# carlos-gg/dl4ds

Measured on AMD Instinct MI355X. Metric: HR samples/s (train step) at 4x 128->512 residual SR, higher is better.
Workload: dtype f32; 1 GPU; configs[1]: net_postupsampling(resnet, spc, scale=4, lr 128x128 -> hr 512x512, 204405 params), MAE, Adam; per_gpu_batch=64, global_batch=64, parallelism=dp1

## Files before the change

dl4ds_amd/csrc/capi.cpp:

```cpp
#include "../../include/dl4ds_hip.h"
#include "graph.h"
#include "runtime.h"
#include "dist.h"
#include "prof.h"
#include <algorithm>
#include <cmath>
#include <cstring>
#include <cstdlib>
#include <mutex>
#include <vector>

Trainer* trainer_create(Graph* g, int loss_kind, const AdamCfg& cfg);
void graph_load_inputs(Graph& g, const float* const* inputs, int n_inputs, int B, bool is_host);
void trainer_evaluate(Trainer& t, const float* const* inputs, int n_inputs, const float* y_true, int B, bool is_host);
void trainer_loss_and_grads(Trainer& t, const float* const* inputs, int n_inputs, const float* y_true, int B, bool is_host,
                            bool reduce_across_ranks);
void trainer_step(Trainer& t, const float* const* inputs, int n_inputs, const float* y_true, int B, bool is_host, float* loss_host);
struct CganTrainer;
CganTrainer* cgan_create(Graph* gen, Graph* disc, int px_loss_kind, float lr, float beta1, float lam);
void cgan_destroy(CganTrainer* t);
void cgan_step(CganTrainer& t, const float* const* gen_inputs, int n_gen_inputs, const float* hr, int B, bool is_host,
               const float* dropout_keep_host, bool apply_update, float* losses_host);
Trainer* cgan_disc_trainer(CganTrainer* t);
Trainer* cgan_gen_trainer(CganTrainer* t);
// ... 169 lines not shown
    API_END
}
int dl4ds_memcpy_d2d(void* dst, const void* src, size_t bytes) {
    API_BEGIN
    HIP_CHECK(hipMemcpyAsync(dst, src, bytes, hipMemcpyDeviceToDevice, S()));
    API_END
}
int dl4ds_memset(void* p, int value, size_t bytes) {
    API_BEGIN
    HIP_CHECK(hipMemsetAsync(p, value, bytes, S()));
    API_END
}
int dl4ds_sync(void) {
    API_BEGIN
    dist_stream_sync(S(), "dl4ds_sync");
    API_END
}
namespace {
__global__ void raise_device_error_kernel(unsigned* word, unsigned code) {
    __hip_atomic_fetch_or(word, code, __ATOMIC_RELAXED, __HIP_MEMORY_SCOPE_SYSTEM);
}
}
int dl4ds_debug_raise_device_error(int code) {
    API_BEGIN
    hipLaunchKernelGGL(raise_device_error_kernel, dim3(1), dim3(1), 0, S(), device_error_word(), (unsigned)code);
    HIP_CHECK(hipGetLastError());
    API_END
}
int dl4ds_event_timer_start(void) {
    API_BEGIN
    HIP_CHECK(hipEventRecord(rt().ev0, S()));
    API_END
}
int dl4ds_event_timer_stop(float* ms) {
    API_BEGIN
    HIP_CHECK(hipEventRecord(rt().ev1, S()));
    HIP_CHECK(hipEventSynchronize(rt().ev1));
    HIP_CHECK(hipEventElapsedTime(ms, rt().ev0, rt().ev1));
    API_END
}

int dl4ds_profile_enable(int on) {
    API_BEGIN
    HIP_CHECK(hipStreamSynchronize(S()));
    prof().reset();
    prof().on = (on != 0);
    API_END
}
int dl4ds_profile_filter(const char* tag_prefix) {
    API_BEGIN
    prof().filter = tag_prefix ? tag_prefix : "";
    API_END
}
int dl4ds_profile_report(char* buf, size_t buflen) {
    API_BEGIN
    const std::string r = prof().report_json(S());
    DL4DS_REQUIRE(r.size() + 1 <= buflen, "profile report buffer too small");
    std::memcpy(buf, r.c_str(), r.size() + 1);
    API_END
}

int dl4ds_op_conv2d_fwd(const float* x, const float* w, const float* b, const float* add, float* y, int N, int H, int W,
                        int Cin, int Cout, int KS, int relu, int d2s_r) {
    API_BEGIN
    TView in = make_view(nc(x), N, H, W, Cin);
    TView out = (d2s_r > 1) ? make_view_d2s(y, N, H, W, Cout, d2s_r) : make_view(y, N, H, W, Cout);
    ConvEpilogue ep;
    ep.bias = b;
    if (add) ep.add = make_view(nc(add), N, H, W, Cout);
    ep.relu = relu;
    conv2d_forward(S(), in, w, KS, out, ep);
    API_END
}
int dl4ds_op_conv2d_epilogue(const float* x, const float* w, const float* b, const float* add, const float* mask, float* y, int N,
                             int H, int W, int Cin, int Cout, int KS, int relu, int accumulate) {
    API_BEGIN
    ConvEpilogue ep;
    ep.bias = b;
    if (add) ep.add = make_view(nc(add), N, H, W, Cout);
    if (mask) ep.mask = make_view(nc(mask), N, H, W, Cout);
    ep.relu = relu;
    ep.accumulate = accumulate;
    conv2d_forward(S(), make_view(nc(x), N, H, W, Cin), w, KS, make_view(y, N, H, W, Cout), ep);
    API_END
}
int dl4ds_op_conv2d_dgrad(const float* dz, const float* w, float* dx, int N, int H, int W, int Cin, int Cout, int KS,
                          int d2s_r, int accumulate) {
    API_BEGIN
    const size_t nw = (size_t)KS * KS * Cin * Cout;
    float* wt = scratch(nw * sizeof(float));
    conv2d_dgrad_weights(S(), w, wt, KS, Cin, Cout);
    TView dzv = (d2s_r > 1) ? make_view_d2s(nc(dz), N, H, W, Cout, d2s_r) : make_view(nc(dz), N, H, W, Cout);
    ConvEpilogue ep;
    ep.accumulate = accumulate;
    conv2d_forward(S(), dzv, wt, KS, make_view(dx, N, H, W, Cin), ep);
    API_END
}
int dl4ds_op_conv2d_wgrad(const float* x, const float* dz, float* dw, int N, int H, int W, int Cin, int Cout, int KS,
                          int d2s_r, int accumulate) {
    API_BEGIN
    TView xv = make_view(nc(x), N, H, W, Cin);
    TView dzv = (d2s_r > 1) ? make_view_d2s(nc(dz), N, H, W, Cout, d2s_r) : make_view(nc(dz), N, H, W, Cout);
    const size_t ws = conv2d_wgrad_workspace_bytes(xv, dzv, KS);
    conv2d_wgrad(S(), xv, dzv, KS, dw, accumulate, nullptr, 0, scratch(ws), ws);
    API_END
}
int dl4ds_op_bias_act_bwd(float* dy, const float* y, float* db, int N, int H, int W, int C) {
    API_BEGIN
    TView dyv = make_view(dy, N, H, W, C);
    TView none{nullptr, 0, 0, 0, 0, 0, 0, 0};
    const size_t ws = bias_grad_workspace_bytes(dyv);
    bias_act_backward(S(), dyv, y ? make_view(nc(y), N, H, W, C) : none, y ? dyv : none, db, 0, scratch(ws), ws);
    API_END
}
int dl4ds_op_conv2d_transpose_fwd(const float* x, const float* w, float* y, int N, int H, int W, int Cin, int Cout,
                                  int KS, int stride, int relu) {
    API_BEGIN
    TView in = make_view(nc(x), N, H, W, Cin);
    TView out = make_view(y, N, H * stride, W * stride, Cout);
    const size_t ws = conv2d_transpose_workspace_bytes(in, out, KS, stride);
    conv2d_transpose_forward(S(), in, w, KS, stride, out, relu, scratch(ws), ws);
    API_END
}
int dl4ds_op_conv2d_transpose_dgrad(const float* dz, const float* w, float* dx, int N, int H, int W, int Cin, int Cout,
                                    int KS, int stride, int accumulate) {
    API_BEGIN
    TView dxv = make_view(dx, N, H, W, Cin);
    TView dzv = make_view(nc(dz), N, H * stride, W * stride, Cout);
    const size_t ws = conv2d_transpose_workspace_bytes(dxv, dzv, KS, stride);
    conv2d_transpose_dgrad(S(), dzv, w, KS, stride, dxv, accumulate, scratch(ws), ws);
    API_END
}
int dl4ds_op_conv2d_transpose_wgrad(const float* x, const float* dz, float* dw, int N, int H, int W, int Cin, int Cout,
                                    int KS, int stride, int accumulate) {
    API_BEGIN
    TView xv = make_view(nc(x), N, H, W, Cin);
    TView dzv = make_view(nc(dz), N, H * stride, W * stride, Cout);
    const size_t ws = conv2d_transpose_workspace_bytes(xv, dzv, KS, stride);
    conv2d_transpose_wgrad(S(), xv, dzv, KS, stride, dw, accumulate, scratch(ws), ws);
    API_END
}
int dl4ds_batch_prepare(const float* hr, const float* pred, const float* stat, const int* idx_host, const int* cy_host,
                        const int* cx_host, float* out_lr, float* out_hr, float* out_stat, int H, int W, int C, int P, int S_,
                        int T, int B, int scale, int psy, int psx, int pin, int static_in_lr) {
    API_BEGIN
    DL4DS_REQUIRE(B > 0 && idx_host && cy_host && cx_host, "batch_prepare: index lists missing");
    const int* d_idx = upload_index_lists(idx_host, cy_host, cx_host, B);
    batch_prepare(S(), hr, pred, stat, d_idx, d_idx + B, d_idx + 2 * B, out_lr, out_hr, out_stat, H, W, C, P, S_, T, B, scale,
                  psy, psx, pin, static_in_lr);
    API_END
}
int dl4ds_batch_prepare_taps(const float* hr, const float* pred, const float* stat, const int* idx_host, const int* cy_host,
                             const int* cx_host, float* out_lr, float* out_hr, float* out_stat, float* scratch_dev, int H, int W,
                             int C, int P, int S_, int T, int B, int scale, int psy, int psx, int pin, int static_in_lr,
                             const dl4ds_tap_axis* dn_patch, const dl4ds_tap_axis* dn_field, const dl4ds_tap_axis* up_field) {
    API_BEGIN
    DL4DS_REQUIRE(B > 0 && idx_host && cy_host && cx_host, "batch_prepare_taps: index lists missing");
    const int* d_idx = upload_index_lists(idx_host, cy_host, cx_host, B);
    auto axes = [](const dl4ds_tap_axis* t, TapAxis* o) -> const TapAxis* {
        if (!t) return nullptr;
        for (int i = 0; i < 2; ++i) { o[i].idx = t[i].idx; o[i].wt = t[i].wt; o[i].k = t[i].k; }
        return o;
    };
    TapAxis a0[2], a1[2], a2[2];
    batch_prepare_taps(S(), hr, pred, stat, d_idx, d_idx + B, d_idx + 2 * B, out_lr, out_hr, out_stat, scratch_dev, H, W, C, P,
                       S_, T, B, scale, psy, psx, pin, static_in_lr, axes(dn_patch, a0), axes(dn_field, a1), axes(up_field, a2));
// ... 803 lines not shown
```

dl4ds_amd/csrc/conv.hip:

```cpp
#include "ops.h"
#include "prof.h"
#include "conv_kernels.h"
#include "conv_cache.h"
#include <algorithm>
#include <mutex>
#include <vector>
#include <cstdlib>

namespace {

constexpr int kLdsBudget = 80 * 1024;

template <int KS, int MT, int NT, int WM, int WN, int KSP = 1>
__global__ void __launch_bounds__(64 * WM * WN * KSP, KSP > 2 ? 1 : 2) conv_igemm_kernel(const ConvParams a) {
    constexpr int TW = 16;
    constexpr int NTHR = 64 * WM * WN * KSP;
    constexpr int BM = WM * MT * 16;
    constexpr int TH = BM / TW;
    constexpr int BN = WN * NT * 16;
    constexpr int BN4 = BN / 4;
    constexpr int PAD = KS / 2;
    constexpr int TWH = TW + KS - 1;
    constexpr int THH = TH + KS - 1;
    constexpr int HPIX = TWH * THH;
// ... 1296 lines not shown
    constexpr bool PF = (CIT == 1 && WCO == 1 && KS <= 3);
    constexpr int TWH = 16 + KS - 1, THH = 8 + KS - 1, HPIX = TWH * THH;
    constexpr int CIB = 16 * CIT, COB = 16 * COT * WCO;
    constexpr int PX = (CIB % 32 == 16) ? CIB : CIB + 16;
    constexpr int PZ = (COB % 32 == 16) ? COB : COB + 16;
    constexpr int WK = 4 / WCO;
    constexpr size_t red_bytes = (size_t)(WK / 2) * WCO * (KS * KS * CIT * COT * 4 + COT) * 64 * sizeof(float);
    static const bool no_rows = exp_env("DL4DS_NO_WGRAD_ROWS") != nullptr;
    constexpr bool ROWS_OK = (KS == 3 || KS == 1 || (KS == 5 && CIT == 1)) && COT == 1;
    const bool rows = ROWS_OK && !no_rows && ((KS == 3 && !PF) || pl.ws);
    const bool ws = rows && pl.ws;
    const size_t lds = rows ? std::max((size_t)(ws ? 2 : 1) * (HPIX * (CIB + 4) + 128 * (COB + 4)) * sizeof(float), red_bytes)
                            : std::max((size_t)(PF ? 2 : 1) * (HPIX * PX + 128 * PZ) * sizeof(float), red_bytes);
    void (*kern)(const WgradParams) = conv_wgrad_kernel<KS, CIT, COT, WCO, PF>;
    static const bool no_pack = exp_env("DL4DS_NO_WGRAD_PACK") != nullptr;
    constexpr bool PACK_OK = ROWS_OK && CIT == 1 && (KS == 3 || KS == 5);
    const bool pack = PACK_OK && ws && p.Cin <= 8 && !no_pack;
    if constexpr (ROWS_OK) {
        if constexpr (KS == 3) {
            if constexpr (PF) { if (rows) kern = conv_wgrad_rows_ws_kernel<CIT, WCO, 3>; }
            else if (rows) kern = ws ? conv_wgrad_rows_ws_kernel<CIT, WCO, 3> : conv_wgrad_rows_kernel<CIT, WCO>;
        } else {
            if (rows) kern = conv_wgrad_rows_ws_kernel<CIT, WCO, KS>;
        }
    }
    if constexpr (PACK_OK) {
        if (pack) kern = conv_wgrad_rows_ws_kernel<1, WCO, KS, true>;
    }
    static std::once_flag once;
    std::call_once(once, [&]() {
        HIP_CHECK(hipFuncSetAttribute(reinterpret_cast<const void*>(conv_wgrad_kernel<KS, CIT, COT, WCO, PF>),
                                      hipFuncAttributeMaxDynamicSharedMemorySize, KS >= 7 ? kLdsMax : kLdsBudget));
        if constexpr (PACK_OK)
            HIP_CHECK(hipFuncSetAttribute(reinterpret_cast<const void*>(conv_wgrad_rows_ws_kernel<1, WCO, KS, true>),
                                          hipFuncAttributeMaxDynamicSharedMemorySize, kLdsMax));
        if constexpr (ROWS_OK) {
            HIP_CHECK(hipFuncSetAttribute(reinterpret_cast<const void*>(conv_wgrad_rows_ws_kernel<CIT, WCO, KS>),
                                          hipFuncAttributeMaxDynamicSharedMemorySize, kLdsMax));
            if constexpr (KS == 3 && !PF)
                HIP_CHECK(hipFuncSetAttribute(reinterpret_cast<const void*>(conv_wgrad_rows_kernel<CIT, WCO>),
                                              hipFuncAttributeMaxDynamicSharedMemorySize, kLdsBudget));
        }
    });
    DL4DS_REQUIRE(lds <= (size_t)((ws || KS >= 7) ? kLdsMax : kLdsBudget), "wgrad tile does not fit in LDS");
    dim3 grid((unsigned)pl.S, (unsigned)cdiv(p.Cout, COB), (unsigned)cdiv(p.Cin, CIB));
    const double px = (double)p.x.N * p.H * p.W;
    ProfScope ps(s, std::string(rows ? "conv_wgrad_rows<" : "conv_wgrad<") + std::to_string(KS) + "," + std::to_string(CIT) +
                        "," + std::to_string(COT) + "," + std::to_string(WCO) + ">",
                 2.0 * px * KS * KS * p.Cin * p.Cout, 4.0 * (px * (p.Cin + p.Cout) + (double)KS * KS * p.Cin * p.Cout));
    DL4DS_LAUNCH(kern, grid, dim3(ws ? 512 : 256), lds, s, p);
    HIP_CHECK(hipGetLastError());
}

template <int KS, int CIT>
void dispatch_wgrad_wco(hipStream_t s, WgradParams& p, const WgradPlan& pl) {
    switch (pl.WCO) {
        case 1: launch_wgrad<KS, CIT, 1, 1>(s, p, pl); break;
        case 2: launch_wgrad<KS, CIT, 1, 2>(s, p, pl); break;
        default: launch_wgrad<KS, CIT, 1, 4>(s, p, pl); break;
    }
}

template <int KS>
void dispatch_wgrad(hipStream_t s, WgradParams& p, const WgradPlan& pl) {
    switch (pl.CIT) {
        case 3: dispatch_wgrad_wco<KS, 3>(s, p, pl); break;
        case 2: dispatch_wgrad_wco<KS, 2>(s, p, pl); break;
        default: dispatch_wgrad_wco<KS, 1>(s, p, pl); break;
    }
}

}

float* conv_splitk_scratch(hipStream_t s, size_t floats) { return splitk_scratch(s, floats); }
void conv_splitk_combine(hipStream_t s, const float* slabs, int S, size_t slab_stride, const ConvParams& p, int N) {
    const size_t total = (size_t)N * p.H * p.W * p.Cout;
    DL4DS_LAUNCH(splitk_combine_kernel, dim3((unsigned)std::min<size_t>(cdivz(total, 256), 4096)), dim3(256), 0, s, slabs, S, slab_stride, p, N);
    HIP_CHECK(hipGetLastError());
}

void conv2d_forward(hipStream_t s, const TView& in, const float* w, int KS, const TView& out,
                    const ConvEpilogue& ep) {
    DL4DS_REQUIRE(in.N == out.N && in.H == out.H && in.W == out.W, "conv2d: stride-1 SAME shapes differ");
    if (conv2d_direct_forward(s, in, w, KS, out, ep)) return;
    if (!exp_env("DL4DS_NO_NARROW") && conv2d_narrow_forward(s, in, w, KS, out, ep)) return;
    DL4DS_REQUIRE(!in.sc && !ep.pool, "conv2d: channel-affine input / pooling partials are only implemented by the direct "
                                     "and narrow-pair kernels (the caller must check conv2d_direct_eligible / conv2d_narrow_pair_ok)");
    if (KS == 3 && conv2d_split_forward(s, in, w, out, ep)) return;
    if (KS == 3 && conv2d_wino_forward(s, in, w, out, ep)) return;
    if (conv2d_gemm_forward(s, in, w, KS, out, ep, 16 * 16)) return;
    if (KS == 1 && exp_env("DL4DS_POINT_FIRST") && conv2d_point_forward(s, in, w, KS, out, ep)) return;
    if (!exp_env("DL4DS_NO_STREAM") && conv2d_stream_forward(s, in, w, KS, out, ep)) return;
    if (conv2d_point_forward(s, in, w, KS, out, ep)) return;
    if (conv2d_gemm_forward(s, in, w, KS, out, ep, 32 * 32)) return;
    ConvParams p;
    p.in = in; p.out = out; p.add = ep.add; p.mask = ep.mask;
    p.w = w; p.bias = ep.bias;
    p.Cin = in.C; p.Cout = out.C; p.H = in.H; p.W = in.W;
    p.relu = ep.relu; p.accumulate = ep.accumulate;
    p.wvec = ((out.C & 3) == 0) && ((((uintptr_t)w) & 15) == 0);
    p.CK = 0; p.TPS = 1; p.tiles_x = p.tiles_y = 0;
    switch (KS) {
        case 1: dispatch_fwd<1>(s, p, in.N); break;
        case 3: dispatch_fwd<3>(s, p, in.N); break;
        case 5: dispatch_fwd<5>(s, p, in.N); break;
        case 7: dispatch_fwd<7>(s, p, in.N); break;
        default: throw Dl4dsError("conv2d: kernel size " + std::to_string(KS) + " not supported (1,3,5,7)");
    }
}

__global__ void __launch_bounds__(256) dgrad_weights_tiled_kernel(const float* __restrict__ w, float* __restrict__ wt, int KK, int Cin,
                                                                  int Cout) {
    __shared__ float tile[32][33];
    const int tp = blockIdx.z;
    const float* src = w + (size_t)(KK - 1 - tp) * Cin * Cout;
    float* dst = wt + (size_t)tp * Cout * Cin;
    const int ci0 = blockIdx.x * 32, co0 = blockIdx.y * 32;
    const int tx = threadIdx.x & 31, ty = threadIdx.x >> 5;
    for (int r = ty; r < 32; r += 8) {
        const int ci = ci0 + r, co = co0 + tx;
        tile[r][tx] = (ci < Cin && co < Cout) ? src[(size_t)ci * Cout + co] : 0.f;
    }
    __syncthreads();
    for (int r = ty; r < 32; r += 8) {
        const int co = co0 + r, ci = ci0 + tx;
        if (co < Cout && ci < Cin) dst[(size_t)co * Cin + ci] = tile[tx][r];
    }
}

__global__ void __launch_bounds__(256) dgrad_weights_batched_kernel(const DgradWeightsJob* __restrict__ jobs, int nj) {
    __shared__ float tile[32][33];
    int j = 0;
    while (j + 1 < nj && (int)blockIdx.x >= jobs[j + 1].block0) ++j;
    const DgradWeightsJob job = jobs[j];
    int b = (int)blockIdx.x - job.block0;
    const int nci = (job.Cin + 31) / 32, nco = (job.Cout + 31) / 32;
    const int bi = b % nci; b /= nci;
    const int bo = b % nco;
    const int tp = b / nco;
    const float* src = job.src + (size_t)(job.KK - 1 - tp) * job.Cin * job.Cout;
    float* dst = job.dst + (size_t)tp * job.Cout * job.Cin;
    const int ci0 = bi * 32, co0 = bo * 32;
    const int tx = threadIdx.x & 31, ty = threadIdx.x >> 5;
    for (int r = ty; r < 32; r += 8) {
        const int ci = ci0 + r, co = co0 + tx;
        tile[r][tx] = (ci < job.Cin && co < job.Cout) ? src[(size_t)ci * job.Cout + co] : 0.f;
    }
    __syncthreads();
    for (int r = ty; r < 32; r += 8) {
        const int co = co0 + r, ci = ci0 + tx;
        if (co < job.Cout && ci < job.Cin) dst[(size_t)co * job.Cin + ci] = tile[tx][r];
    }
}
int dgrad_weights_job_blocks(int KK, int Cin, int Cout) { return cdiv(Cin, 32) * cdiv(Cout, 32) * KK; }
void conv2d_dgrad_weights_batched(hipStream_t s, const DgradWeightsJob* jobs_dev, int nj, int blocks) {
    if (nj == 0 || blocks == 0) return;
    ProfScope ps(s, "dgrad_weights_batched", 0.0, 0.0);
    DL4DS_LAUNCH(dgrad_weights_batched_kernel, dim3(blocks), dim3(256), 0, s, jobs_dev, nj);
    HIP_CHECK(hipGetLastError());
}

void conv2d_dgrad_weights(hipStream_t s, const float* w, float* wt, int KS, int Cin, int Cout) {
    const size_t total = (size_t)KS * KS * Cin * Cout;
    ProfScope ps(s, "dgrad_weights", 0.0, 8.0 * (double)total);
    if ((size_t)Cin * Cout >= 4096 && Cin >= 16 && Cout >= 16) {
        DL4DS_LAUNCH(dgrad_weights_tiled_kernel, dim3(cdiv(Cin, 32), cdiv(Cout, 32), KS * KS), dim3(256), 0, s, w, wt, KS * KS,
                           Cin, Cout);
    } else {
        const int blocks = (int)std::min<size_t>(cdivz(total, 256), 2048);
        DL4DS_LAUNCH(dgrad_weights_kernel, dim3(blocks), dim3(256), 0, s, w, wt, KS * KS, Cin, Cout);
    }
    HIP_CHECK(hipGetLastError());
}

static TView channel_slice(const TView& x, int c0, int c1) {
    TView v = x;
    v.p = x.p + c0; v.C = c1 - c0; v.cp = v.C;
    v.vec = ((v.C & 3) == 0) && ((x.ld & 3) == 0) && ((((uintptr_t)v.p) & 15) == 0);
    return v;
}
static int narrow_wgrad_split_slabs(const TView& x, const TView& dz, int KS) {
    static const bool off = exp_env("DL4DS_NO_WGRAD_SPLIT") != nullptr;
    if (off || KS != 3 || x.C <= 8 || x.C > 16 || dz.C > 8 || x.sc || x.d2s > 1 || dz.d2s > 1 || !dz.vec) return 0;
    if (conv2d_direct_wgrad_slabs(x, dz, KS) || exp_env("DL4DS_NO_NARROW")) return 0;
    return conv2d_narrow_wgrad_slabs(channel_slice(x, 0, 8), dz, KS);
}

size_t conv2d_wgrad_workspace_bytes(const TView& x, const TView& dz, int KS) {
    const size_t slab = ((size_t)KS * KS * x.C * dz.C + dz.C) * sizeof(float);
    if (const int ds = conv2d_direct_wgrad_slabs(x, dz, KS)) return (size_t)ds * slab;
    const size_t general = (size_t)plan_wgrad(x, dz, KS).S * slab;
// ... 70 lines not shown
```

dl4ds_amd/csrc/conv_split.hip:

```cpp
#include "ops.h"
#include "prof.h"
#include "launch.h"
#include "conv_cache.h"
#include <algorithm>
#include <cstdlib>
#include <string>
#include <vector>
#include <cstdio>

namespace {

typedef float f32x4 __attribute__((ext_vector_type(4)));
typedef __bf16 bf16x8 __attribute__((ext_vector_type(8)));
typedef __bf16 bf16x4 __attribute__((ext_vector_type(4)));
typedef unsigned u32x4 __attribute__((ext_vector_type(4)));
typedef int i32x4 __attribute__((ext_vector_type(4)));
constexpr int OOB = (int)0x7fffff80, RSRC3 = 0x00020000;

constexpr int SPX = 32;
constexpr int HPX = SPX + 2;
constexpr int PIXB = 288;
constexpr int ROWB = HPX * PIXB;
constexpr int RPIX = 52;
constexpr int REDF = 5 * SPX * RPIX;
constexpr int NMW = 12, NHW = 4;
constexpr int NTHREADS = 64 * (NMW + NHW);
constexpr size_t LDS_BYTES = 3 * ROWB + 2 * REDF * sizeof(float) + 48 * sizeof(float);

struct SplitParams {
    TView in, out, add, mask;
    const float* bias;
    const u32x4* frag;
    int cin0, Cin;
    int Cout, H, W;
    int nchunk;
    int nsx, nsy, R;
    int nitems;
    int relu, old;
    int final_pass;
    unsigned long long* trace;
};

__host__ __device__ inline int split_unit(int w, int i) {
    if (w < NMW) return i < 2 ? 2 * (w & 3) + i : -1;
    return (i == 0 && w - NMW < 3) ? 8 : -1;
}
__host__ __device__ inline int split_tile(int w) { return w < NMW ? w >> 2 : w - NMW; }

__device__ __forceinline__ u32x4 split_filter_entry(const float* __restrict__ w, int CinTot, int cin0, int Cout, int e) {
    int i = e;
    const int lane = i & 63; i >>= 6;
    const int form = i % 2; i /= 2;
    const int ky = i % 3; i /= 3;
    const int ui = i % 2; i /= 2;
    const int wv = i % (NMW + NHW);
    const int chunk = i / (NMW + NHW);
    const int u = split_unit(wv, ui), kx = u / 3, c = u % 3, ct = split_tile(wv);
    const int kq = lane >> 4, co = chunk * 48 + ct * 16 + (lane & 15);
    const int part = (kq < 2) ? (form == 0 ? 0 : 2) : (form == 0 ? 1 : 0);
    bf16x8 v;
#pragma unroll
    for (int j = 0; j < 8; ++j) {
        const int ci = cin0 + 16 * c + 8 * (kq & 1) + j;
        const float x = (u >= 0 && ci < CinTot && co < Cout) ? w[((size_t)(ky * 3 + kx) * CinTot + ci) * Cout + co] : 0.f;
        const __bf16 h = (__bf16)x;
        const float r1 = x - (float)h;
        const __bf16 m = (__bf16)r1;
        const __bf16 l = (__bf16)(r1 - (float)m);
        v[j] = part == 0 ? h : (part == 1 ? m : l);
    }
    u32x4 o;
    __builtin_memcpy(&o, &v, 16);
    return o;
}

__global__ void __launch_bounds__(256) split_filter_kernel(const float* __restrict__ w, u32x4* __restrict__ frag, int CinTot, int cin0,
                                                           int Cout, int nchunk, int total) {
    const int e = blockIdx.x * 256 + threadIdx.x;
    if (e >= total) return;
    (void)nchunk;
    frag[e] = split_filter_entry(w, CinTot, cin0, Cout, e);
}

struct SplitFilterJob { const float* w; u32x4* frag; int Cin, Cout, per_pass, total, first; };
__global__ void __launch_bounds__(256) split_filter_batched_kernel(const FilterJobs<SplitFilterJob> jobs) {
    int k = 0;
#pragma unroll 1
    while (k + 1 < jobs.n && (int)blockIdx.x >= jobs.j[k + 1].first) ++k;
    const int e_all = ((int)blockIdx.x - jobs.j[k].first) * 256 + (int)threadIdx.x;
    if (e_all >= jobs.j[k].total) return;
    const int per_pass = jobs.j[k].per_pass, pass = e_all / per_pass;
    jobs.j[k].frag[e_all] = split_filter_entry(jobs.j[k].w, jobs.j[k].Cin, pass * 48, jobs.j[k].Cout, e_all - pass * per_pass);
}

__device__ __forceinline__ void split4(const float4 x, bf16x4& h, bf16x4& m, bf16x4& l) {
    const float xs[4] = {x.x, x.y, x.z, x.w};
    unsigned hb[4], mb[4], lb[4];
#pragma unroll
    for (int j = 0; j < 4; ++j) {
        hb[j] = __float_as_uint(xs[j]) & 0xffff0000u;
        const float r1 = xs[j] - __uint_as_float(hb[j]);
        mb[j] = __float_as_uint(r1) & 0xffff0000u;
        lb[j] = __float_as_uint(r1 - __uint_as_float(mb[j]));
    }
    unsigned hp[2], mp[2], lp[2];
#pragma unroll
    for (int j = 0; j < 2; ++j) {
        hp[j] = __builtin_amdgcn_perm(hb[2 * j + 1], hb[2 * j], 0x07060302u);
        mp[j] = __builtin_amdgcn_perm(mb[2 * j + 1], mb[2 * j], 0x07060302u);
        lp[j] = __builtin_amdgcn_perm(lb[2 * j + 1], lb[2 * j], 0x07060302u);
    }
    __builtin_memcpy(&h, hp, 8); __builtin_memcpy(&m, mp, 8); __builtin_memcpy(&l, lp, 8);
}

__device__ __forceinline__ void split_mma9(const bf16x8 (&A)[3][2], const bf16x8 (&b)[3], f32x4& N, f32x4& M, f32x4& O) {
    N = __builtin_amdgcn_mfma_f32_16x16x32_bf16(A[0][1], b[2], N, 0, 0, 0);
    M = __builtin_amdgcn_mfma_f32_16x16x32_bf16(A[1][1], b[2], M, 0, 0, 0);
    O = __builtin_amdgcn_mfma_f32_16x16x32_bf16(A[2][1], b[2], O, 0, 0, 0);
    N = __builtin_amdgcn_mfma_f32_16x16x32_bf16(A[0][0], b[1], N, 0, 0, 0);
    M = __builtin_amdgcn_mfma_f32_16x16x32_bf16(A[1][0], b[1], M, 0, 0, 0);
    O = __builtin_amdgcn_mfma_f32_16x16x32_bf16(A[2][0], b[1], O, 0, 0, 0);
    N = __builtin_amdgcn_mfma_f32_16x16x32_bf16(A[0][0], b[0], N, 0, 0, 0);
    M = __builtin_amdgcn_mfma_f32_16x16x32_bf16(A[1][0], b[0], M, 0, 0, 0);
    O = __builtin_amdgcn_mfma_f32_16x16x32_bf16(A[2][0], b[0], O, 0, 0, 0);
}
__device__ __forceinline__ void split_fetch(const unsigned char* rb, int b1, int b2, int b3, int o, bf16x8 (&b)[3]) {
    b[2] = *reinterpret_cast<const bf16x8*>(rb + b3 + o);
    b[1] = *reinterpret_cast<const bf16x8*>(rb + b2 + o);
    b[0] = *reinterpret_cast<const bf16x8*>(rb + b1 + o);
}

#ifdef SPLIT_TRACE
#define SPLIT_STAMP(k) do { const unsigned _n = (unsigned)__builtin_readcyclecounter(); _tw[(k) - 1] += _n - _t0; _t0 = _n; if ((k) == 2) ++_tw[2]; } while (0)
#define SPLIT_TRACE_DECL unsigned _tw[3] = {0, 0, 0}; unsigned _t0 = 0
#define SPLIT_TRACE_START _t0 = (unsigned)__builtin_readcyclecounter()
#define SPLIT_TRACE_END do { if (p.trace && lane == 0) { unsigned long long* tr = p.trace + ((size_t)blockIdx.x * (NMW + NHW) + wave) * 4; tr[0] = _tw[0]; tr[1] = _tw[1]; tr[3] = _tw[2]; } } while (0)
#else
#define SPLIT_STAMP(k) do { } while (0)
#define SPLIT_TRACE_DECL
#define SPLIT_TRACE_START
#define SPLIT_TRACE_END
#endif
template <bool OLD, bool ADD, bool MASK>
__global__ void __launch_bounds__(NTHREADS) conv_split_kernel(const SplitParams p) {
    extern __shared__ __attribute__((aligned(16))) unsigned char smem[];
    unsigned char* rowbuf = smem;
    float* red = reinterpret_cast<float*>(smem + 3 * ROWB);
    float* lbias = red + 2 * REDF;
    const int tid = threadIdx.x, lane = tid & 63, wave = tid >> 6;
    const int chunk = blockIdx.x % p.nchunk;
    const int slot = blockIdx.x / p.nchunk, nslots = gridDim.x / p.nchunk;
    const int n16 = lane & 15, kq = lane >> 4;
    const int boff1 = n16 * PIXB + (kq >> 1) * 96 + (kq & 1) * 16;
    const int boff2 = n16 * PIXB + ((kq >> 1) ^ 1) * 96 + (kq & 1) * 16;
    const int boff3 = n16 * PIXB + (kq >> 1) * 192 + (kq & 1) * 16;
    const int ct = split_tile(wave);
    const int rslot = wave < NMW ? (wave & 3) : 4;
    const int rdoff = (rslot * SPX + n16) * RPIX + (ct < 3 ? ct : 0) * 16 + kq * 4;
    SPLIT_TRACE_DECL;
    if (tid < 48) lbias[tid] = (p.bias && p.final_pass && chunk * 48 + tid < p.Cout) ? p.bias[chunk * 48 + tid] : 0.f;

    if (wave < NMW) {
        bf16x8 A[2][3][2];
        {
            const u32x4* f = p.frag + ((size_t)(chunk * (NMW + NHW) + wave) * 12) * 64 + lane;
#pragma unroll
            for (int i = 0; i < 12; ++i) {
                const u32x4 v = f[(size_t)i * 64];
                __builtin_memcpy(&A[i / 6][(i / 2) % 3][i % 2], &v, 16);
            }
        }
        int uo[2];
#pragma unroll
        for (int i = 0; i < 2; ++i) {
            const int u = split_unit(wave, i);
            uo[i] = __builtin_amdgcn_readfirstlane((u / 3) * PIXB + (u % 3) * 32);
        }
        const int epx = tid / 12, eq = tid - epx * 12;
        const int co = chunk * 48 + eq * 4;
        const bool e_el = tid < SPX * 12 && co < p.Cout;
        const int out_ys = (p.out.d2s > 1 ? p.out.d2s * p.out.d2s : 1) * p.W * p.out.ld * 4;
        const int add_ys = ADD ? (p.add.d2s > 1 ? p.add.d2s * p.add.d2s : 1) * p.W * p.add.ld * 4 : 0;
        const int mask_ys = MASK ? (p.mask.d2s > 1 ? p.mask.d2s * p.mask.d2s : 1) * p.W * p.mask.ld * 4 : 0;
        for (int item = slot; item < p.nitems; item += nslots) {
            int q = item;
            const int sx = q % p.nsx; q /= p.nsx;
            const int sy = q % p.nsy;
            const int n = q / p.nsy;
            const int y_lo = sy * p.R, y_hi = min(y_lo + p.R, p.H);
            const int exg = sx * SPX + epx;
            const bool e_ok = e_el && exg < p.W;
            const int ooff = e_ok ? (int)(view_off(p.out, 0, 0, exg, co) * 4) : OOB;
            const int aoff = (ADD && e_ok) ? (int)(view_off(p.add, 0, 0, exg, co) * 4) : OOB;
            const int moff = (MASK && e_ok) ? (int)(view_off(p.mask, 0, 0, exg, co) * 4) : OOB;
            const __amdgpu_buffer_rsrc_t rs_out = __builtin_amdgcn_make_buffer_rsrc(p.out.p + (size_t)n * p.out.nstride, 0, 0x7fffff00, RSRC3);
            const __amdgpu_buffer_rsrc_t rs_add = __builtin_amdgcn_make_buffer_rsrc(
                const_cast<float*>(ADD ? p.add.p + (size_t)n * p.add.nstride : p.out.p), 0, 0x7fffff00, RSRC3);
            const __amdgpu_buffer_rsrc_t rs_mask = __builtin_amdgcn_make_buffer_rsrc(
                const_cast<float*>(MASK ? p.mask.p + (size_t)n * p.mask.nstride : p.out.p), 0, 0x7fffff00, RSRC3);
            i32x4 ov = {0, 0, 0, 0}, av = {0, 0, 0, 0}, mv = {0, 0, 0, 0};
            auto request = [&](int yo) __attribute__((always_inline)) {
                const int eoff = (yo >= y_lo && yo < y_hi && ooff != OOB) ? 0 : OOB;
                if constexpr (OLD) ov = __builtin_amdgcn_raw_buffer_load_b128(rs_out, (eoff | ooff) + (eoff == 0 ? yo * out_ys : 0), 0, 0);
                if constexpr (ADD) av = __builtin_amdgcn_raw_buffer_load_b128(rs_add, (eoff | aoff) + (eoff == 0 ? yo * add_ys : 0), 0, 0);
                if constexpr (MASK) mv = __builtin_amdgcn_raw_buffer_load_b128(rs_mask, (eoff | moff) + (eoff == 0 ? yo * mask_ys : 0), 0, 0);
            };
            auto finish = [&](int yo, int buf) __attribute__((always_inline)) {
                const int eoff = (yo >= y_lo && yo < y_hi && ooff != OOB) ? 0 : OOB;
                const float* r0 = red + buf * REDF + epx * RPIX + eq * 4;
                const float4 a0 = *reinterpret_cast<const float4*>(r0);
                const float4 a1 = *reinterpret_cast<const float4*>(r0 + SPX * RPIX);
                const float4 a2 = *reinterpret_cast<const float4*>(r0 + 2 * SPX * RPIX);
                const float4 a3 = *reinterpret_cast<const float4*>(r0 + 3 * SPX * RPIX);
                const float4 a4 = *reinterpret_cast<const float4*>(r0 + 4 * SPX * RPIX);
                float4 v = make_float4(((a0.x + a1.x) + (a2.x + a3.x)) + a4.x, ((a0.y + a1.y) + (a2.y + a3.y)) + a4.y,
                                       ((a0.z + a1.z) + (a2.z + a3.z)) + a4.z, ((a0.w + a1.w) + (a2.w + a3.w)) + a4.w);
                float4 o = make_float4(0.f, 0.f, 0.f, 0.f), r = o, mk = o;
                if constexpr (OLD) __builtin_memcpy(&o, &ov, 16);
                if constexpr (ADD) __builtin_memcpy(&r, &av, 16);
                if constexpr (MASK) __builtin_memcpy(&mk, &mv, 16);
                if (OLD && p.old == 1) { v.x += o.x; v.y += o.y; v.z += o.z; v.w += o.w; }
                if (p.final_pass) {
                    const float4 b4 = *reinterpret_cast<const float4*>(lbias + eq * 4);
                    v.x += b4.x; v.y += b4.y; v.z += b4.z; v.w += b4.w;
                    if (ADD) { v.x += r.x; v.y += r.y; v.z += r.z; v.w += r.w; }
                    if (p.relu) { v.x = fmaxf(v.x, 0.f); v.y = fmaxf(v.y, 0.f); v.z = fmaxf(v.z, 0.f); v.w = fmaxf(v.w, 0.f); }
                    if (MASK) { v.x = mk.x > 0.f ? v.x : 0.f; v.y = mk.y > 0.f ? v.y : 0.f; v.z = mk.z > 0.f ? v.z : 0.f; v.w = mk.w > 0.f ? v.w : 0.f; }
                    if (OLD && p.old == 2) { v.x += o.x; v.y += o.y; v.z += o.z; v.w += o.w; }
                }
                i32x4 vi;
                __builtin_memcpy(&vi, &v, 16);
                __builtin_amdgcn_raw_buffer_store_b128(vi, rs_out, (eoff | ooff) + (eoff == 0 ? yo * out_ys : 0), 0, 0);
            };
            f32x4 acc[3][2];
#pragma unroll
            for (int a = 0; a < 3; ++a)
#pragma unroll
                for (int pt = 0; pt < 2; ++pt) acc[a][pt] = (f32x4){0.f, 0.f, 0.f, 0.f};
            int y = y_lo - 1;
            __syncthreads();
            SPLIT_TRACE_START;
            bf16x8 bA[3], bB[3];
            split_fetch(rowbuf, boff1, boff2, boff3, uo[0], bA);
            auto row = [&](int K, f32x4 (&N)[2], f32x4 (&M)[2], f32x4 (&O)[2]) __attribute__((always_inline)) {
                const unsigned char* rb = rowbuf + K * ROWB;
                __builtin_amdgcn_sched_barrier(0);
                split_fetch(rb, boff1, boff2, boff3, uo[0] + 16 * PIXB, bB);
                __builtin_amdgcn_sched_barrier(0);
                split_mma9(A[0], bA, N[0], M[0], O[0]);
                __builtin_amdgcn_sched_barrier(0);
                if (wave < 6) {
                    finish(y - 2, (y - 1) & 1);
                    request(y - 1);
                }
                __builtin_amdgcn_sched_barrier(0);
                split_fetch(rb, boff1, boff2, boff3, uo[1], bA);
                __builtin_amdgcn_sched_barrier(0);
                split_mma9(A[0], bB, N[1], M[1], O[1]);
                __builtin_amdgcn_sched_barrier(0);
                split_fetch(rb, boff1, boff2, boff3, uo[1] + 16 * PIXB, bB);
                __builtin_amdgcn_sched_barrier(0);
                split_mma9(A[1], bA, N[0], M[0], O[0]);
                __builtin_amdgcn_sched_barrier(0);
                split_fetch(rowbuf + ((K + 1) % 3) * ROWB, boff1, boff2, boff3, uo[0], bA);
                __builtin_amdgcn_sched_barrier(0);
                split_mma9(A[1], bB, N[1], M[1], O[1]);
                __builtin_amdgcn_sched_barrier(0);
                float* rd = red + (y & 1) * REDF + rdoff;
#pragma unroll
                for (int pt = 0; pt < 2; ++pt) {
                    *reinterpret_cast<f32x4*>(rd + pt * 16 * RPIX) = O[pt];
                    O[pt] = (f32x4){0.f, 0.f, 0.f, 0.f};
                }
                SPLIT_STAMP(1);
                __syncthreads();
                SPLIT_STAMP(2);
                ++y;
            };
            while (y <= y_hi) {
                row(0, acc[0], acc[1], acc[2]);
                if (y > y_hi) break;
                row(1, acc[2], acc[0], acc[1]);
                if (y > y_hi) break;
                row(2, acc[1], acc[2], acc[0]);
            }
            if (wave < 6) finish(y - 2, (y - 1) & 1);
        }
        SPLIT_TRACE_END;
        return;
    }

    const int hid = tid - 64 * NMW;
    constexpr int NH = 64 * NHW;
    const bool hunit = ct < 3;
    bf16x8 A[3][2];
    {
        const u32x4* f = p.frag + ((size_t)(chunk * (NMW + NHW) + wave) * 12) * 64 + lane;
#pragma unroll
        for (int i = 0; i < 6; ++i) {
            const u32x4 v = f[(size_t)i * 64];
            __builtin_memcpy(&A[i / 2][i % 2], &v, 16);
        }
    }
    const int uo = 2 * PIXB + 2 * 32;
    const int in_ys = (p.in.d2s > 1 ? p.in.d2s * p.in.d2s : 1) * p.W * p.in.ld * 4;
    int spx[2], sq[2];
    bool s_el[2];
#pragma unroll
    for (int k = 0; k < 2; ++k) {
        const int e = hid + k * NH;
        spx[k] = e / 12; sq[k] = e - spx[k] * 12; s_el[k] = e < HPX * 12;
    }
    for (int item = slot; item < p.nitems; item += nslots) {
        int q = item;
        const int sx = q % p.nsx; q /= p.nsx;
// ... 2 lines not shown
        const int x0 = sx * SPX, y_lo = sy * p.R, y_hi = min(y_lo + p.R, p.H);
        int soff[2];
#pragma unroll
        for (int k = 0; k < 2; ++k) {
            const int sxg = x0 - 1 + spx[k], sc = p.cin0 + sq[k] * 4;
            const bool s_ok = s_el[k] && sxg >= 0 && sxg < p.W && sc < p.Cin;
            soff[k] = s_ok ? (int)(view_off(p.in, 0, 0, sxg, sc) * 4) : OOB;
        }
        const __amdgpu_buffer_rsrc_t rs_in = __builtin_amdgcn_make_buffer_rsrc(p.in.p + (size_t)n * p.in.nstride, 0, 0x7fffff00, RSRC3);

        i32x4 nxt[2];
        auto load_row = [&](int y) __attribute__((always_inline)) {
            const bool ok = y >= 0 && y < p.H;
#pragma unroll
            for (int k = 0; k < 2; ++k) nxt[k] = __builtin_amdgcn_raw_buffer_load_b128(rs_in, (ok && soff[k] != OOB) ? soff[k] + y * in_ys : OOB, 0, 0);
        };
        auto stage_row = [&](int buf) __attribute__((always_inline)) {
#pragma unroll
            for (int k = 0; k < 2; ++k) {
                if (s_el[k]) {
                    float4 v;
                    __builtin_memcpy(&v, &nxt[k], 16);
                    bf16x4 h, m, l;
                    split4(v, h, m, l);
                    unsigned char* d = rowbuf + buf * ROWB + spx[k] * PIXB + sq[k] * 8;
                    *reinterpret_cast<bf16x4*>(d) = h;
                    *reinterpret_cast<bf16x4*>(d + 96) = m;
                    *reinterpret_cast<bf16x4*>(d + 192) = l;
                }
            }
        };
        f32x4 acc[3][2];
#pragma unroll
        for (int a = 0; a < 3; ++a)
#pragma unroll
            for (int pt = 0; pt < 2; ++pt) acc[a][pt] = (f32x4){0.f, 0.f, 0.f, 0.f};
        int y = y_lo - 1;
        load_row(y);
        stage_row(0);
        load_row(y + 1);
        stage_row(1);
        load_row(y + 2);
        __syncthreads();
        SPLIT_TRACE_START;
        auto row = [&](int K, f32x4 (&N)[2], f32x4 (&M)[2], f32x4 (&O)[2]) __attribute__((always_inline)) {
            if (hunit) {
                const unsigned char* rb = rowbuf + K * ROWB;
                bf16x8 bA[3];
                __builtin_amdgcn_s_setprio(3);
#pragma unroll
                for (int pt = 0; pt < 2; ++pt) {
                    __builtin_amdgcn_sched_barrier(0);
                    split_fetch(rb, boff1, boff2, boff3, uo + pt * 16 * PIXB, bA);
                    split_mma9(A, bA, N[pt], M[pt], O[pt]);
                }
                __builtin_amdgcn_sched_barrier(0);
                __builtin_amdgcn_s_setprio(0);
                float* rd = red + (y & 1) * REDF + rdoff;
#pragma unroll
                for (int pt = 0; pt < 2; ++pt) {
                    *reinterpret_cast<f32x4*>(rd + pt * 16 * RPIX) = O[pt];
                    O[pt] = (f32x4){0.f, 0.f, 0.f, 0.f};
                }
            }
            __builtin_amdgcn_sched_barrier(0);
            stage_row((K + 2) % 3);
            load_row(y + 3);
            SPLIT_STAMP(1);
            __syncthreads();
            SPLIT_STAMP(2);
            ++y;
        };
        while (y <= y_hi) {
            row(0, acc[0], acc[1], acc[2]);
            if (y > y_hi) break;
            row(1, acc[2], acc[0], acc[1]);
            if (y > y_hi) break;
            row(2, acc[1], acc[2], acc[0]);
        }
    }
    SPLIT_TRACE_END;
}

template <bool OLD, bool ADD, bool MASK>
void launch_one(hipStream_t s, const SplitParams& p, int grid) {
    static bool once = false;
    if (!once) {
        HIP_CHECK(hipFuncSetAttribute(reinterpret_cast<const void*>(conv_split_kernel<OLD, ADD, MASK>), hipFuncAttributeMaxDynamicSharedMemorySize,
                                      (int)LDS_BYTES));
        once = true;
    }
    DL4DS_LAUNCH((conv_split_kernel<OLD, ADD, MASK>), dim3(grid), dim3(NTHREADS), LDS_BYTES, s, p);
    HIP_CHECK(hipGetLastError());
}
void launch_form(hipStream_t s, const SplitParams& p, int grid) {
    const int f = (p.old ? 4 : 0) | (p.add.p ? 2 : 0) | (p.mask.p ? 1 : 0);
    switch (f) {
        case 0: launch_one<false, false, false>(s, p, grid); break;
        case 1: launch_one<false, false, true>(s, p, grid); break;
        case 2: launch_one<false, true, false>(s, p, grid); break;
        case 3: launch_one<false, true, true>(s, p, grid); break;
        case 4: launch_one<true, false, false>(s, p, grid); break;
        case 5: launch_one<true, false, true>(s, p, grid); break;
        case 6: launch_one<true, true, false>(s, p, grid); break;
        default: launch_one<true, true, true>(s, p, grid); break;
    }
}

int cu_count() {
    static const int n = [] {
        int dev = 0, v = 0;
        HIP_CHECK(hipGetDevice(&dev));
        HIP_CHECK(hipDeviceGetAttribute(&v, hipDeviceAttributeMultiprocessorCount, dev));
        return v;
    }();
    return n;
}

struct SplitFilterKey {
    int Cin, Cout, per_pass, passes;
    bool operator==(const SplitFilterKey& o) const { return Cin == o.Cin && Cout == o.Cout && per_pass == o.per_pass && passes == o.passes; }
};
typedef DerivedFilterCache<SplitFilterKey, SplitFilterJob> SplitFilterCache;
SplitFilterCache& split_filters() { static SplitFilterCache c(1 << 18); return c; }

}

void split_filters_invalidate(const float* lo, const float* hi) { split_filters().invalidate(lo, hi); }
void split_filters_release(const float* lo, const float* hi) { split_filters().release(lo, hi); }

void split_filters_refresh(hipStream_t s, const float* lo, const float* hi, int kind) {
    split_filters().refresh(
        s, lo, hi, kind,
        [](const SplitFilterCache::Entry& e, SplitFilterJob& j) {
            const SplitFilterKey& k = e.key;
            j = SplitFilterJob{e.w, reinterpret_cast<u32x4*>(e.buf), k.Cin, k.Cout, k.per_pass, k.per_pass * k.passes, 0};
            return cdiv(j.total, 256);
        },
        [&](const FilterJobs<SplitFilterJob>& jobs) {
            ProfScope ps(s, "split_filters", 0.0, 16.0 * jobs.total * 256);
            DL4DS_LAUNCH(split_filter_batched_kernel, dim3(jobs.total), dim3(256), 0, s, jobs);
            HIP_CHECK(hipGetLastError());
        });
}

bool conv2d_split_forward(hipStream_t s, const TView& in, const float* w, const TView& out, const ConvEpilogue& ep) {
    const char* force = test_env("DL4DS_SPLIT_FORCE");
    if (getenv("DL4DS_NO_SPLIT")) return false;
    const bool every_shape = getenv("DL4DS_SPLIT") != nullptr || force != nullptr;
    if (in.sc || ep.pool) return false;
    if (!in.vec || !out.vec || (in.C & 3) || (out.C & 3) || (ep.add.p && !ep.add.vec) || (ep.mask.p && !ep.mask.vec)) return false;
    if ((((uintptr_t)ep.bias) & 15) != 0) return false;
    if (in.C <= 32 || (in.C > 48 && in.C % 48 != 0)) return false;
    if (out.C <= 32 || cdiv(out.C, 32) * 32 < cdiv(out.C, 48) * 48) return false;
    const int passes = cdiv(in.C, 48);
    if (!every_shape && (passes > 1 || out.C > 48)) return false;
    if (passes > 1 && ep.accumulate) return false;
    if (ep.add.p && (ep.add.C != out.C)) return false;
    auto span = [](const TView& v) { const size_t r = std::max(v.d2s, 1); return (size_t)(v.H + 2) * v.W * r * r * v.ld * 4; };
    if (span(in) >= (1ull << 31) || span(out) >= (1ull << 31) || (ep.add.p && span(ep.add) >= (1ull << 31)) ||
        (ep.mask.p && span(ep.mask) >= (1ull << 31))) return false;
    SplitParams p;
    p.in = in; p.out = out; p.add = ep.add; p.mask = ep.mask; p.bias = ep.bias;
    p.Cin = in.C; p.Cout = out.C; p.H = in.H; p.W = in.W;
    p.nchunk = cdiv(out.C, 48);
    p.nsx = cdiv(in.W, SPX);
    p.R = in.H <= 32 ? in.H : 32;
    if (in.H > 16 && (long)p.nsx * cdiv(in.H, p.R) * in.N * cdiv(out.C, 48) < (long)cu_count()) p.R = 16;
    if (const char* r = test_env("DL4DS_SPLIT_R")) p.R = std::max(1, std::min(atoi(r), in.H));
    p.nsy = cdiv(in.H, p.R);
    const long items = (long)p.nsx * p.nsy * in.N;
    if (items >= (1l << 24) || (!force && items * p.nchunk < (long)cu_count())) return false;
    p.nitems = (int)items;
    p.relu = ep.relu;
    const double px = (double)in.N * in.H * in.W;
    const double fl = 2.0 * px * 9.0 * in.C * out.C;
    ProfScope ps(s, std::string("conv_split<3,3>") + (test_env("DL4DS_SPLIT_TAG_FORMS") ? std::string("f") + std::to_string((ep.accumulate ? 4 : 0) | (ep.add.p ? 2 : 0) | (ep.mask.p ? 1 : 0)) + "c" + std::to_string(in.C) + "_" + std::to_string(out.C) : std::string()), fl,
                 4.0 * (px * (in.C + out.C * (1 + (ep.add.p ? 1 : 0) + (ep.mask.p ? 1 : 0) + (ep.accumulate ? 1 : 0))) + 9.0 * in.C * out.C), fl);
    const int per_pass = p.nchunk * (NMW + NHW) * 12 * 64;
    bool need_frag = true;
    u32x4* frag = reinterpret_cast<u32x4*>(
        split_filters().lookup(s, w, SplitFilterKey{in.C, out.C, per_pass, passes}, (size_t)per_pass * passes * 4, need_frag));
    int grid = std::min((int)std::min<long>(items, cu_count()), cu_count()) * 1;
    grid = std::max(1, grid / p.nchunk) * p.nchunk;
    if (grid > cu_count()) grid = (cu_count() / p.nchunk) * p.nchunk;
    if (force && atoi(force) > 0) grid = std::min(grid, atoi(force) * p.nchunk);
    p.trace = nullptr;
    static unsigned long long* trace_buf = nullptr;
    const bool tracing = test_env("DL4DS_SPLIT_TRACE") != nullptr;
    if (tracing) {
        if (!trace_buf) HIP_CHECK(hipMalloc((void**)&trace_buf, 256 * (NMW + NHW) * 4 * 8));
        HIP_CHECK(hipMemsetAsync(trace_buf, 0, 256 * (NMW + NHW) * 4 * 8, s));
        p.trace = trace_buf;
    }
    for (int ps_ = 0; ps_ < passes; ++ps_) {
        p.cin0 = ps_ * 48;
        p.frag = frag + (size_t)per_pass * ps_;
        if (need_frag) {
            DL4DS_LAUNCH(split_filter_kernel, dim3(cdiv(per_pass, 256)), dim3(256), 0, s, w, const_cast<u32x4*>(p.frag), in.C, p.cin0, out.C, p.nchunk,
                         per_pass);
            HIP_CHECK(hipGetLastError());
        }
        p.final_pass = ps_ == passes - 1;
        p.old = (ps_ > 0) ? 1 : (ep.accumulate ? 2 : 0);
        if (!p.final_pass) { p.add.p = nullptr; p.mask.p = nullptr; } else { p.add = ep.add; p.mask = ep.mask; }
        launch_form(s, p, grid);
    }
    if (tracing) {
        HIP_CHECK(hipStreamSynchronize(s));
        std::vector<unsigned long long> h((size_t)grid * (NMW + NHW) * 4);
        HIP_CHECK(hipMemcpy(h.data(), trace_buf, h.size() * 8, hipMemcpyDeviceToHost));
        for (int w = 0; w < NMW + NHW; ++w) {
            double a = 0, b = 0, c = 0, r = 0;
            for (int g = 0; g < grid; ++g) { a += h[((size_t)g * (NMW + NHW) + w) * 4]; b += h[((size_t)g * (NMW + NHW) + w) * 4 + 1]; c += h[((size_t)g * (NMW + NHW) + w) * 4 + 2]; r += h[((size_t)g * (NMW + NHW) + w) * 4 + 3]; }
            fprintf(stderr, "conv_split trace wave %d: per row: work %.0f, barrier wait %.0f cycles (%.0f rows per workgroup; Cin %d Cout %d passes %d)\n",
                    w, a / r, b / r, r / grid, in.C, out.C, passes); (void)c;
        }
    }
    return true;
}
```

dl4ds_amd/csrc/conv_wino.hip:

```cpp
#include "conv_wino_kernel.h"
#include "conv_wino4_kernel.h"
#include "conv_cache.h"

namespace {

int wino_cu_count() {
    static const int n = [] {
        int dev = 0, v = 0;
        HIP_CHECK(hipGetDevice(&dev));
        HIP_CHECK(hipDeviceGetAttribute(&v, hipDeviceAttributeMultiprocessorCount, dev));
        return v;
    }();
    return n;
}

__device__ __forceinline__ float wino_filter_value(const float* __restrict__ w, int Cin, int Cout, int KQ, int NT, int nchunk, int idx) {
    const int F = 16 * KQ * NT;
    const int j = idx & 3, lane = (idx >> 2) & 63;
    int r = idx >> 8;
    const int f4 = r % (F / 4); r /= F / 4;
    const int xi = r & 3; r >>= 2;
    const int chunk = r % nchunk, pass = r / nchunk;
    const int f = 4 * f4 + j;
    const int nu = f / (4 * KQ * NT), ks = (f / NT) % (4 * KQ), cb = f % NT;
// ... 93 lines not shown
    wino_filters().invalidate(lo, hi);
    split_filters_invalidate(lo, hi);
}

void derived_filters_release(const float* lo, const float* hi) {
    split_filters_release(lo, hi);
    wino_filters().release(lo, hi);
}

void derived_filters_refresh(hipStream_t s, const float* lo, const float* hi, int kind) {
    wino_filters().refresh(
        s, lo, hi, kind,
        [](const WinoFilterCache::Entry& e, WinoFilterJob& j) {
            const WinoFilterKey& k = e.key;
            j = WinoFilterJob{e.w, e.buf, k.Cin, k.Cout, k.KQ, k.NT, k.nchunk, (int)e.floats, 0, k.f44};
            return cdiv(j.total, WINO_FILTER_PER_BLOCK);
        },
        [&](const FilterJobs<WinoFilterJob>& jobs) {
            ProfScope ps(s, "wino_filters", 0.0, 4.0 * jobs.total * WINO_FILTER_PER_BLOCK);
            DL4DS_LAUNCH(wino_filter_batched_kernel, dim3(jobs.total), dim3(256), 0, s, jobs);
            HIP_CHECK(hipGetLastError());
        });
    split_filters_refresh(s, lo, hi, kind);
}

static bool conv2d_wino4_forward(hipStream_t s, const TView& in, const float* w, const TView& out, const ConvEpilogue& ep, int KQ, int cpass,
                                 const char* force) {
    const char* f44 = test_env("DL4DS_WINO_F44");
    const bool forced = f44 && f44[0] == 'f';
    if (!forced && (out.C % 32) != 0) return false;
    if (!forced && in.C % cpass != 0 && in.C > cpass) return false;
    const int NT = 2;
    const int passes = cdiv(in.C, cpass);
    const int full_epi = (ep.add.p ? WINO_ADD : 0) | (ep.mask.p ? WINO_MASK : 0) | (ep.accumulate ? WINO_OLDA : 0);
    auto span = [](const TView& v) { const size_t r = std::max(v.d2s, 1); return (size_t)24 * v.W * r * r * v.ld * 4; };
    if (span(in) >= (1ull << 31) || span(out) >= (1ull << 31)) return false;
    WinoParams wp;
    ConvParams& p = wp.c;
    p.in = in; p.out = out; p.add = ep.add; p.mask = ep.mask;
    p.w = w; p.bias = ep.bias;
    p.Cin = in.C; p.Cout = out.C; p.H = in.H; p.W = in.W;
    p.relu = ep.relu; p.accumulate = ep.accumulate;
    wp.nchunk = cdiv(out.C, 16 * NT);
    wp.tgx = cdiv(in.W, 16);
    wp.tgy = cdiv(in.H, 16);
    wp.m_tgx = div_magic(wp.tgx);
    wp.m_tgy = div_magic(wp.tgy);
    const long ntg = (long)wp.tgx * wp.tgy * in.N;
    if (ntg >= (1l << 20)) return false;
    wp.ntg = (int)ntg;
    wp.per_xcd = cdiv(wp.ntg, 8);
    const int SXmax = std::max(wino_cu_count() / 8, 1);
    if (wp.nchunk > SXmax) return false;
    int SX = (SXmax / wp.nchunk) * wp.nchunk;
    if (force && atoi(force) > 0) SX = std::min(SX, atoi(force) * wp.nchunk);
    if (!force && (long)wp.per_xcd * wp.nchunk < 4l * SX) return false;
    const double px = (double)in.N * in.H * in.W;
    const double issued = 2.0 * (px / 16.0) * 36.0 * (16.0 * KQ * passes) * (16.0 * NT * wp.nchunk) +
                          (px / 16.0) * (2.0 * 154.0 * 4.0 * in.C * wp.nchunk / 4.0 + 124.0 * out.C * passes);
    ProfScope ps(s, "conv_wino4<" + std::to_string(KQ) + "," + std::to_string(NT) + ">", issued,
                 4.0 * (px * (in.C + out.C * (1 + (ep.add.p ? 1 : 0) + (ep.mask.p ? 1 : 0) + (ep.accumulate ? 1 : 0))) + 9.0 * in.C * out.C),
                 2.0 * px * 9.0 * in.C * out.C);
    const size_t per_pass = (size_t)wp.nchunk * 4 * (36 * KQ * NT) * 64;
    const int total = (int)(per_pass * passes);
    bool need = true;
    float* const u = wino_filter_lookup(s, w, in.C, out.C, KQ, NT, wp.nchunk, total, need, 1);
    if (need) {
        DL4DS_LAUNCH(wino4_filter_kernel, dim3(std::min(cdiv(total, 256), 2048)), dim3(256), 0, s, w, u, in.C, out.C, KQ, NT,
                     wp.nchunk, total);
        HIP_CHECK(hipGetLastError());
    }
    for (int ps_ = 0; ps_ < passes; ++ps_) {
        const bool last = ps_ == passes - 1;
        wp.cin0 = ps_ * cpass;
        wp.u = u + per_pass * ps_;
        wp.first = ps_ == 0;
        p.relu = last ? ep.relu : 0;
        const int epi = passes == 1 ? full_epi : ((ps_ ? WINO_OLDF : 0) | (last ? full_epi : 0));
        if (KQ == 2) launch_wino4_22(s, wp, SX, epi); else launch_wino4_32(s, wp, SX, epi);
    }
    return true;
}

bool conv2d_wino_forward(hipStream_t s, const TView& in, const float* w, const TView& out, const ConvEpilogue& ep) {
    const bool off = getenv("DL4DS_NO_WINOGRAD") != nullptr;
    const char* force = test_env("DL4DS_WINO_FORCE");
    if (off) return false;
    if (in.sc || ep.pool) return false;
    if (!in.vec || !out.vec || (in.C & 3) || (out.C & 3) || (ep.add.p && !ep.add.vec) || (ep.mask.p && !ep.mask.vec)) return false;
    if ((((uintptr_t)ep.bias) & 15) != 0) return false;
    if (in.C < 24 || out.C < 24) return false;
    auto same_layout = [](const TView& u, const TView& v) { return u.ld == v.ld && u.d2s == v.d2s && u.W == v.W && u.cp == v.cp; };
    if (ep.add.p && !same_layout(ep.add, out)) return false;
    if (ep.mask.p && !same_layout(ep.mask, out)) return false;
    auto span = [](const TView& v) { const size_t r = std::max(v.d2s, 1); return (size_t)8 * v.W * r * r * v.ld * 4; };
    if (span(in) >= (1ull << 31) || span(out) >= (1ull << 31)) return false;
    int KQ, cpass;
    if (in.C <= 32) { KQ = 2; cpass = 32; }
    else if (in.C <= 48) { KQ = 3; cpass = 48; }
    else if (in.C % 48 == 0) { KQ = 3; cpass = 48; }
    else if (in.C % 32 == 0) { KQ = 2; cpass = 32; }
    else return false;
    const int passes = cdiv(in.C, cpass);
    if (passes > 1 && ep.accumulate) return false;
    const int full_epi = (ep.add.p ? WINO_ADD : 0) | (ep.mask.p ? WINO_MASK : 0) | (ep.accumulate ? WINO_OLDA : 0);
    if (!wino_epi_built(full_epi) || (passes > 1 && !wino_epi_built(full_epi | WINO_OLDF))) return false;
    if (test_env("DL4DS_WINO_F44") && conv2d_wino4_forward(s, in, w, out, ep, KQ, cpass, force)) return true;
    const int NT = (cdiv(out.C, 32) * 32 < cdiv(out.C, 48) * 48) ? 2 : 3;
    WinoParams wp;
    ConvParams& p = wp.c;
    p.in = in; p.out = out; p.add = ep.add; p.mask = ep.mask;
    p.w = w; p.bias = ep.bias;
    p.Cin = in.C; p.Cout = out.C; p.H = in.H; p.W = in.W;
    p.relu = ep.relu; p.accumulate = ep.accumulate;
    wp.nchunk = cdiv(out.C, 16 * NT);
    wp.tgx = cdiv(in.W, 16);
    wp.tgy = cdiv(in.H, 4);
    wp.m_tgx = div_magic(wp.tgx);
    wp.m_tgy = div_magic(wp.tgy);
    const long ntg = (long)wp.tgx * wp.tgy * in.N;
    if (ntg >= (1l << 20)) return false;
    wp.ntg = (int)ntg;
    wp.per_xcd = cdiv(wp.ntg, 8);
    const int SXmax = std::max(2 * wino_cu_count() / 8, 1);
    if (wp.nchunk > SXmax) return false;
    int SX = (SXmax / wp.nchunk) * wp.nchunk;
    if (force && atoi(force) > 0) SX = std::min(SX, atoi(force) * wp.nchunk);
    if (!force && (long)wp.per_xcd * wp.nchunk < 4l * SX) return false;
    const double px = (double)in.N * in.H * in.W;
    const double issued = 2.0 * (px / 4.0) * 16.0 * (16.0 * KQ * passes) * (16.0 * NT * wp.nchunk) +
                          (px / 4.0) * (32.0 * in.C * wp.nchunk + 24.0 * out.C * passes);
    ProfScope ps(s, "conv_wino<" + std::to_string(KQ) + "," + std::to_string(NT) + ">", issued,
                 4.0 * (px * (in.C + out.C * (1 + (ep.add.p ? 1 : 0) + (ep.mask.p ? 1 : 0) + (ep.accumulate ? 1 : 0))) + 9.0 * in.C * out.C),
                 2.0 * px * 9.0 * in.C * out.C);
    const size_t per_pass = (size_t)wp.nchunk * 4 * (16 * KQ * NT) * 64;
    const int total = (int)(per_pass * passes);
    bool need = true;
    float* const u = wino_filter_lookup(s, w, in.C, out.C, KQ, NT, wp.nchunk, total, need);
    if (need) {
        DL4DS_LAUNCH(wino_filter_kernel, dim3(std::min(cdiv(total, 256), 2048)), dim3(256), 0, s, w, u, in.C, out.C, KQ, NT,
                           wp.nchunk, total);
        HIP_CHECK(hipGetLastError());
    }
    for (int ps_ = 0; ps_ < passes; ++ps_) {
        const bool last = ps_ == passes - 1;
        wp.cin0 = ps_ * cpass;
        wp.u = u + per_pass * ps_;
        wp.first = ps_ == 0;
        p.relu = last ? ep.relu : 0;
        const int epi = passes == 1 ? full_epi : ((ps_ ? WINO_OLDF : 0) | (last ? full_epi : 0));
        if (KQ == 2) {
            if (NT == 2) launch_wino_22(s, wp, SX, epi); else launch_wino_23(s, wp, SX, epi);
        } else {
            if (NT == 2) launch_wino_32(s, wp, SX, epi); else launch_wino_33(s, wp, SX, epi);
        }
    }
    return true;
}
```

dl4ds_amd/csrc/conv_wino_kernel.h:

```cpp
#pragma once
#include "ops.h"
#include "prof.h"
#include "conv_kernels.h"
#include <algorithm>
#include <mutex>
#include <string>
#include <vector>

struct WinoParams {
    ConvParams c;
    int cin0;
    const float* u;
    int first;
    int nchunk;
    int ntg, per_xcd;
    int tgx, tgy;
    unsigned m_tgx, m_tgy;
#ifdef WINO_TRACE
    unsigned long long* trace;
#endif
};

enum : int {
    WINO_OLDF = 1,
    WINO_ADD = 2,
    WINO_MASK = 4,
    WINO_OLDA = 8,
};
inline bool wino_epi_built(int e) { return e == 0 || e == 1 || e == 2 || e == 3 || e == 4 || e == 5 || e == 8 || e == 12; }

void launch_wino_22(hipStream_t s, WinoParams& wp, int SX, int epi);
void launch_wino_23(hipStream_t s, WinoParams& wp, int SX, int epi);
void launch_wino_32(hipStream_t s, WinoParams& wp, int SX, int epi);
void launch_wino_33(hipStream_t s, WinoParams& wp, int SX, int epi);

namespace wino {

typedef int i32x4_t __attribute__((ext_vector_type(4)));
typedef float f32x2 __attribute__((ext_vector_type(2)));

__device__ __forceinline__ f32x4 sub4(const f32x4 a, const f32x4 b) {
    f32x2 lo, hi;
    const f32x2 alo = __builtin_shufflevector(a, a, 0, 1), ahi = __builtin_shufflevector(a, a, 2, 3);
    const f32x2 blo = __builtin_shufflevector(b, b, 0, 1), bhi = __builtin_shufflevector(b, b, 2, 3);
    asm("v_pk_add_f32 %0, %1, %2 neg_lo:[0,1] neg_hi:[0,1]" : "=v"(lo) : "v"(alo), "v"(blo));
    asm("v_pk_add_f32 %0, %1, %2 neg_lo:[0,1] neg_hi:[0,1]" : "=v"(hi) : "v"(ahi), "v"(bhi));
    return __builtin_shufflevector(lo, hi, 0, 1, 2, 3);
}

struct PkConsts { f32x2 neg1; };
__device__ __forceinline__ PkConsts pk_consts() {
    float m = -1.f;
    asm volatile("" : "+v"(m));
    PkConsts c;
    c.neg1 = (f32x2){m, m};
    return c;
}
__device__ __forceinline__ f32x2 pk_add(const f32x2 a, const f32x2 b) { return a + b; }
__device__ __forceinline__ f32x2 pk_fma(const f32x2 b, const f32x2 s, const f32x2 c) { return __builtin_elementwise_fma(b, s, c); }
__device__ __forceinline__ f32x2 pk_sub(const PkConsts& k, const f32x2 a, const f32x2 b) { return __builtin_elementwise_fma(b, k.neg1, a); }
__device__ __forceinline__ f32x2 lo2(const f32x4 a) { return __builtin_shufflevector(a, a, 0, 1); }
__device__ __forceinline__ f32x2 hi2(const f32x4 a) { return __builtin_shufflevector(a, a, 2, 3); }
__device__ __forceinline__ f32x4 cat4(const f32x2 l, const f32x2 h) { return __builtin_shufflevector(l, h, 0, 1, 2, 3); }
__device__ __forceinline__ f32x4 add4(const f32x4 a, const f32x4 b) {
#ifdef WINO_SCALAR_VALU
    return a + b;
#else
    return cat4(pk_add(lo2(a), lo2(b)), pk_add(hi2(a), hi2(b)));
#endif
}
__device__ __forceinline__ f32x4 subp4(const PkConsts& k, const f32x4 a, const f32x4 b) {
#ifdef WINO_SCALAR_VALU
    return a - b;
#else
    return cat4(pk_sub(k, lo2(a), lo2(b)), pk_sub(k, hi2(a), hi2(b)));
#endif
}
__device__ __forceinline__ f32x4 fma4(const f32x4 b, const f32x2 s, const f32x4 c) {
#ifdef WINO_SCALAR_VALU
    return c + s[0] * b;
#else
    return cat4(pk_fma(lo2(b), s, lo2(c)), pk_fma(hi2(b), s, hi2(c)));
#endif
}

__device__ __forceinline__ void view_strides(const TView& v, size_t& sy, size_t& sx) {
    const int r = v.d2s > 1 ? v.d2s : 1;
    sx = (size_t)r * v.ld;
    sy = (size_t)r * (size_t)(v.W * r) * v.ld;
}

template <int KQ, int NT>
struct Wino2Geom {
    static constexpr int CK = 16 * KQ, Q4 = 4 * KQ, CO = 16 * NT, NQ = 4 * NT;
    static constexpr int SP = Q4 + 1;
    static constexpr int HW = 18, HH = 6, HPIX = HW * HH;
    static constexpr int NSLOT = HPIX * SP, NCH = (NSLOT + 63) / 64, RAWS = NCH * 64;
    static constexpr int SIT = (NCH + 3) / 4;
    static constexpr int PP = CO + 8;
    static constexpr int P = 8 * 16 * PP;
    static constexpr int TAB = (SIT + (SIT + 3) / 4) * 256;
    static constexpr size_t LDS_BYTES = (size_t)(2 * RAWS * 4 + P + TAB) * 4;
    static_assert(2 * LDS_BYTES <= 160 * 1024, "two workgroups per CU");
};

__device__ __forceinline__ int wino2_col_of_tile(int ty, int tx) { return ty ? tx + 4 : (tx < 4 ? tx : tx + 8); }

template <int KQ, int NT, int EPI>
__global__ void __launch_bounds__(256, 2) conv_wino2_kernel(const WinoParams wp) {
    typedef Wino2Geom<KQ, NT> GM;
    const ConvParams& a = wp.c;
    constexpr int Q4 = GM::Q4, CO = GM::CO, NQ = GM::NQ, SP = GM::SP, PP = GM::PP;
    constexpr int HW = GM::HW, HH = GM::HH, HPIX = GM::HPIX, SIT = GM::SIT, NCH = GM::NCH;
    constexpr int OOB = (int)0xffffff00u;
    constexpr int RSRC3 = 0x00020000;
    constexpr bool OLDF = (EPI & WINO_OLDF) != 0, ADD = (EPI & WINO_ADD) != 0, MASK = (EPI & WINO_MASK) != 0, OLDA = (EPI & WINO_OLDA) != 0;
    extern __shared__ __attribute__((aligned(16))) float lds[];
    float* const raw = lds;
    float* const Pb = lds + 2 * GM::RAWS * 4;

    const int tid = threadIdx.x, lane = tid & 63, wave = __builtin_amdgcn_readfirstlane(tid >> 6), l15 = lane & 15, lq = lane >> 4;
    const int xcd = blockIdx.x & 7, slot = blockIdx.x >> 3, SX = gridDim.x >> 3;
    const int nsub = SX / wp.nchunk;
    const int chunk = slot % wp.nchunk, sub = slot / wp.nchunk;
    const int n0 = chunk * CO;
    const int tg_lo = xcd * wp.per_xcd, tg_hi = min(wp.ntg, tg_lo + wp.per_xcd);
    int tg = tg_lo + sub;
    if (sub >= nsub || tg >= tg_hi) return;

    size_t isy, isx;
    view_strides(a.in, isy, isx);
    int* const tab = reinterpret_cast<int*>(Pb + GM::P) + tid;
    {
        unsigned hyx[(SIT + 3) / 4];
#pragma unroll
        for (int u = 0; u < (SIT + 3) / 4; ++u) hyx[u] = 0;
#pragma unroll
        for (int u = 0; u < SIT; ++u) {
            const int L = (4 * u + wave) * 64 + lane;
            const int p = L / SP, q = L - p * SP;
            const int cq = wp.cin0 + 4 * q;
            const int hy = p / HW, hx = p - hy * HW;
            const bool ok = q < Q4 && p < HPIX && cq < a.Cin;
            tab[u * 256] = ok ? (int)((hy * isy + hx * isx + view_chan_off(a.in, cq)) * 4) : OOB;
            hyx[u >> 2] |= (unsigned)(ok ? (hy | (hx << 3)) : 0) << (8 * (u & 3));
        }
#pragma unroll
        for (int u = 0; u < (SIT + 3) / 4; ++u) tab[(SIT + u) * 256] = (int)hyx[u];
    }
    struct Item { int n, y0, x0; };
    auto decode = [&](int t) {
        const int q = fast_div(t, wp.m_tgx);
        const int bx = t - q * wp.tgx;
        const int n = fast_div(q, wp.m_tgy);
        const int by = q - n * wp.tgy;
        Item it;
        it.n = n; it.y0 = by * 4; it.x0 = bx * 16;
        return it;
    };
    typedef __attribute__((address_space(3))) void* lds_ptr_t;
    auto stage_issue = [&](const Item& it, int buf) __attribute__((always_inline)) {
        const int ylo = max(0, 1 - it.y0), yhi = min(HH, a.H + 1 - it.y0);
        const int xlo = max(0, 1 - it.x0), xhi = min(HW, a.W + 1 - it.x0);
        int so[SIT];
#pragma unroll
        for (int u = 0; u < SIT; ++u) so[u] = tab[u * 256];
        if (ylo | xlo | (yhi - HH) | (xhi - HW)) {
            asm volatile("" ::: "memory");
#pragma unroll
            for (int u = 0; u < SIT; ++u) {
                const unsigned w = (unsigned)tab[(SIT + (u >> 2)) * 256];
                const int b = (int)((w >> (8 * (u & 3))) & 255u);
                const int hy = b & 7, hx = b >> 3;
                so[u] = (hy >= ylo && hy < yhi && hx >= xlo && hx < xhi) ? so[u] : OOB;
            }
        }
        const long org = (long)((size_t)it.n * a.in.nstride) + (long)(it.y0 - 1) * (long)isy + (long)(it.x0 - 1) * (long)isx;
        const __amdgpu_buffer_rsrc_t rs = __builtin_amdgcn_make_buffer_rsrc(
            const_cast<char*>(reinterpret_cast<const char*>(a.in.p)) + org * 4, 0, 0x7fffff00, RSRC3);
#if defined(__HIP_DEVICE_COMPILE__)
        float* const dst = raw + buf * (GM::RAWS * 4) + wave * 256;
#pragma unroll
        for (int u = 0; u < SIT; ++u)
            if (4 * u + wave < NCH)
                __builtin_amdgcn_raw_ptr_buffer_load_lds(rs, (lds_ptr_t)(dst + u * 1024), 16, so[u], 0, 0, 0);
#else
        (void)rs; (void)so; (void)buf;
#endif
    };

    const int ra = wave == 0 ? 0 : (wave == 2 ? 2 : 1);
    const int rb = wave == 0 ? 2 : (wave == 1 ? 2 : (wave == 2 ? 1 : 3));
    const float sg1 = wave == 1 ? 1.f : -1.f;
    const f32x2 sg = {sg1, sg1};
    const PkConsts pkc = pk_consts();
    const int k_ty = (l15 >= 4 && l15 < 12) ? 1 : 0;
    const int k_tx = k_ty ? l15 - 4 : (l15 < 4 ? l15 : l15 - 8);
    const int k_base = ((2 * k_ty * HW + 2 * k_tx) * SP + lq) * 4;
    const int k_a = k_base + ra * HW * SP * 4, k_b = k_base + rb * HW * SP * 4;
// ... 100 lines not shown
                __builtin_amdgcn_sched_barrier(0);
                rowt(0); loadc(kq + 1, 1);
                mfmas(kq, 1);
                if (kq == 0 && has_next) {
                    nxt = decode(ntg);
#ifndef WINO_NO_LOAD
                    stage_issue(nxt, buf ^ 1);
#endif
                }
                __builtin_amdgcn_sched_barrier(0);
                rowt(1); loadc(kq + 1, 2);
                mfmas(kq, 2);
                __builtin_amdgcn_sched_barrier(0);
                rowt(2); loadc(kq + 1, 3);
                mfmas(kq, 3);
                rowt(3); colt();
            }
            __builtin_amdgcn_sched_barrier(0);
            mfmas(KQ - 1, 1);
            if (KQ == 1 && has_next) {
                nxt = decode(ntg);
#ifndef WINO_NO_LOAD
                stage_issue(nxt, buf ^ 1);
#endif
            }
            __builtin_amdgcn_sched_barrier(0);
            mfmas(KQ - 1, 2);
            __builtin_amdgcn_sched_barrier(0);
            mfmas(KQ - 1, 0);
#pragma unroll
            for (int cb = 0; cb < NT; ++cb) {
                const f32x4 s12 = add4(acc[1][cb], acc[2][cb]);
                acc[2][cb] = subp4(pkc, acc[1][cb], acc[2][cb]);
                acc[1][cb] = s12;
            }
            __builtin_amdgcn_sched_barrier(0);
            mfmas(KQ - 1, 3);
#pragma unroll
            for (int cb = 0; cb < NT; ++cb) acc[0][cb] = add4(acc[0][cb], acc[1][cb]);
            __builtin_amdgcn_sched_barrier(0);
        }
        WT(2);
        f32x4 R0[NT], R1[NT];
#pragma unroll
        for (int cb = 0; cb < NT; ++cb) {
            R0[cb] = acc[0][cb];
            R1[cb] = add4(acc[3][cb], acc[2][cb]);
        }
        if (want_bias && wave == 1) {
#pragma unroll
            for (int cb = 0; cb < NT; ++cb) {
                const f32x4 b4 = *reinterpret_cast<const f32x4*>(a.bias + min(n0 + 16 * cb + 4 * lq, bias_max));
                R0[cb] = add4(R0[cb], b4);
                R1[cb] = add4(R1[cb], b4);
            }
        }
#pragma unroll
        for (int cb = 0; cb < NT; ++cb) {
            *reinterpret_cast<f32x4*>(pwr + 16 * cb) = R0[cb];
            *reinterpret_cast<f32x4*>(pwr + 16 * PP + 16 * cb) = R1[cb];
        }
        WT(3);
        asm volatile("s_waitcnt vmcnt(0)" ::: "memory");
        WT(4);
        __syncthreads();
        WT(5);
#ifndef WINO_NO_C
        {
            const int ymax = min(4, a.H - cur.y0), xmax = min(16, a.W - cur.x0);
            int dv[ND];
#pragma unroll
            for (int u = 0; u < ND; ++u) dv[u] = dvo[u];
            if ((ymax - 4) | (xmax - 16)) {
                asm volatile("" ::: "memory");
#pragma unroll
                for (int u = 0; u < ND; ++u) {
                    const int pix = (tid + 256 * u) / NQ;
                    dv[u] = ((pix >> 4) < ymax && (pix & 15) < xmax) ? dvo[u] : OOB;
                }
            }
            const size_t pb_ = cur.y0 * osy + cur.x0 * osx;
            const __amdgpu_buffer_rsrc_t ro = __builtin_amdgcn_make_buffer_rsrc(
                reinterpret_cast<char*>(a.out.p) + ((size_t)cur.n * a.out.nstride + pb_) * 4, 0, 0x7fffff00, RSRC3);
            i32x4_t e_old[(OLDF || OLDA) ? ND : 1], e_add[ADD ? ND : 1], e_mask[MASK ? ND : 1];
            if (OLDF || OLDA) {
#pragma unroll
                for (int u = 0; u < ND; ++u) e_old[u] = __builtin_amdgcn_raw_buffer_load_b128(ro, dv[u], 0, 0);
            }
            if (ADD) {
                const __amdgpu_buffer_rsrc_t ra_ = __builtin_amdgcn_make_buffer_rsrc(
                    reinterpret_cast<char*>(a.add.p) + ((size_t)cur.n * a.add.nstride + pb_) * 4, 0, 0x7fffff00, RSRC3);
#pragma unroll
                for (int u = 0; u < ND; ++u) e_add[u] = __builtin_amdgcn_raw_buffer_load_b128(ra_, dv[u], 0, 0);
            }
            if (MASK) {
                const __amdgpu_buffer_rsrc_t rm = __builtin_amdgcn_make_buffer_rsrc(
                    reinterpret_cast<char*>(a.mask.p) + ((size_t)cur.n * a.mask.nstride + pb_) * 4, 0, 0x7fffff00, RSRC3);
#pragma unroll
                for (int u = 0; u < ND; ++u) e_mask[u] = __builtin_amdgcn_raw_buffer_load_b128(rm, dv[u], 0, 0);
            }
#pragma unroll
            for (int u = 0; u < ND; ++u) {
                const float* p = Pb + (prd[u] & 0x3fffffff);
                const f32x4 r0 = *reinterpret_cast<const f32x4*>(p);
                const f32x4 r1 = *reinterpret_cast<const f32x4*>(p + 2 * 16 * PP);
                const f32x4 r2 = *reinterpret_cast<const f32x4*>(p + 4 * 16 * PP);
                const float sgn = __builtin_bit_cast(float, 0x3f800000 | ((prd[u] << 1) & 0x80000000));
                f32x4 r = fma4(add4(r1, r2), (f32x2){sgn, sgn}, r0);
                if (OLDF) r = add4(r, __builtin_bit_cast(f32x4, e_old[u]));
                if (ADD) r = add4(r, __builtin_bit_cast(f32x4, e_add[u]));
                r[0] = fmaxf(r[0], floor_v); r[1] = fmaxf(r[1], floor_v); r[2] = fmaxf(r[2], floor_v); r[3] = fmaxf(r[3], floor_v);
                if (MASK) {
                    const f32x4 m = __builtin_bit_cast(f32x4, e_mask[u]);
                    r[0] = m[0] > 0.f ? r[0] : 0.f; r[1] = m[1] > 0.f ? r[1] : 0.f;
                    r[2] = m[2] > 0.f ? r[2] : 0.f; r[3] = m[3] > 0.f ? r[3] : 0.f;
                }
                if (OLDA) r = add4(r, __builtin_bit_cast(f32x4, e_old[u]));
                __builtin_amdgcn_raw_buffer_store_b128(__builtin_bit_cast(i32x4_t, r), ro, dv[u], 0, 0);
            }
        }
#endif
        WT(6);
#ifdef WINO_TRACE
        tr[0] += 1ull << 48;
#endif
        if (!has_next) break;
        cur = nxt;
        tg = ntg;
        buf ^= 1;
        __syncthreads();
        WT(7);
    }
    (void)prev;
#ifdef WINO_TRACE
    if (wp.trace && lane == 0)
        for (int q = 0; q < 8; ++q) wp.trace[((size_t)blockIdx.x * 4 + wave) * 8 + q] = tr[q];
#endif
}

template <int KQ, int NT, int EPI>
void launch_one(hipStream_t s, WinoParams& wp, int SX) {
#ifdef WINO_TRACE
    static unsigned long long* trace_buf = nullptr;
    static int trace_n = 0;
    wp.trace = nullptr;
    if (trace_n < 3) {
        if (!trace_buf) HIP_CHECK(hipMalloc((void**)&trace_buf, (size_t)1024 * 32 * 8));
        HIP_CHECK(hipMemsetAsync(trace_buf, 0, (size_t)1024 * 32 * 8, s));
        wp.trace = trace_buf;
    }
#endif
    {
        typedef Wino2Geom<KQ, NT> G2;
        static std::once_flag once2;
        std::call_once(once2, [&]() {
            HIP_CHECK(hipFuncSetAttribute(reinterpret_cast<const void*>(conv_wino2_kernel<KQ, NT, EPI>),
                                          hipFuncAttributeMaxDynamicSharedMemorySize, (int)G2::LDS_BYTES));
        });
        DL4DS_LAUNCH((conv_wino2_kernel<KQ, NT, EPI>), dim3(8 * SX), dim3(256), G2::LDS_BYTES, s, wp);
        HIP_CHECK(hipGetLastError());
#ifdef WINO_TRACE
        if (wp.trace) {
            ++trace_n;
            HIP_CHECK(hipStreamSynchronize(s));
            std::vector<unsigned long long> h((size_t)8 * SX * 32);
            HIP_CHECK(hipMemcpy(h.data(), trace_buf, h.size() * 8, hipMemcpyDeviceToHost));
            static const char* nm[8] = {"prologue", "issue", "K", "writeP", "landed", "bar1", "C", "bar2"};
            for (int wv = 0; wv < 4; wv += 3) {
                double sum[8] = {0}, its = 0;
                int nwg = 0;
                for (int b = 0; b < 8 * SX; ++b) {
                    const unsigned long long* t = &h[((size_t)b * 4 + wv) * 8];
                    const double it = (double)(t[0] >> 48);
                    if (it == 0) continue;
                    ++nwg; its += it;
                    for (int q = 0; q < 8; ++q) sum[q] += (double)(q == 0 ? (t[0] & ((1ull << 48) - 1)) : t[q]);
                }
                if (!nwg) continue;
                fprintf(stderr, "wino2<%d,%d,%d> wave %d: %d workgroups, %.1f iterations each; cycles: prologue %.0f | per iteration", KQ, NT, EPI,
                        wv, nwg, its / nwg, sum[0] / nwg);
                double tot = 0;
                for (int q = 1; q < 8; ++q) { fprintf(stderr, " %s %.0f", nm[q], sum[q] / its); tot += sum[q] / its; }
                fprintf(stderr, " = %.0f\n", tot);
            }
        }
#endif
    }
}

template <int KQ, int NT>
void launch_shape(hipStream_t s, WinoParams& wp, int SX, int epi) {
    switch (epi) {
        case 0: launch_one<KQ, NT, 0>(s, wp, SX); break;
        case 1: launch_one<KQ, NT, 1>(s, wp, SX); break;
        case 2: launch_one<KQ, NT, 2>(s, wp, SX); break;
        case 3: launch_one<KQ, NT, 3>(s, wp, SX); break;
        case 4: launch_one<KQ, NT, 4>(s, wp, SX); break;
        case 5: launch_one<KQ, NT, 5>(s, wp, SX); break;
        case 8: launch_one<KQ, NT, 8>(s, wp, SX); break;
        case 12: launch_one<KQ, NT, 12>(s, wp, SX); break;
        default: throw Dl4dsError("conv_wino: epilogue form " + std::to_string(epi) + " is not built");
    }
}

}
```

dl4ds_amd/csrc/graph.h:

```cpp
#pragma once
#include "ops.h"
#include <memory>
#include <string>
#include <vector>

struct Graph;

struct GTensor {
    int H = 0, W = 0, C = 0;
    int nmul = 1;
    bool requires_grad = true;
    bool is_input = false;
    bool dep_grad_input = false;
    float* data = nullptr;
    float* grad = nullptr;
    bool grad_written = false;
    int n_conv_in = 0, n_other = 0;
    int n_add_in = 0;
    int n_masking = 0;
    int n_concat_in = 0;
    int n_fused_add = 0;
    bool two_add_inplace = false;
    int n_pool_in = 0, n_convt_in = 0;
    bool relu_out = false;
    const float* pending_add = nullptr;
    TView pending_view{};
    int alias_of = -1, alias_coff = 0, alias_ld = 0;
    int alias_parent = -1;
    bool galias = false;
    bool grad_masked = false;
    size_t per_sample() const { return (size_t)nmul * H * W * C; }
};

struct GParam {
    size_t offset = 0, n = 0;
    bool grad_written = false;
};

struct BwdCtx {
    int B;
    int b_off, b_cnt;
    bool param_grads;
    bool input_grads;
};

struct GOp {
    virtual ~GOp() {}
    virtual void forward(Graph& g, int B, bool training) = 0;
    virtual void backward(Graph& g, const BwdCtx& c) = 0;
    virtual size_t workspace_bytes(Graph& g, int B) { return 0; }
    virtual size_t saved_floats_per_sample(Graph& g) { return 0; }
    float* saved = nullptr;
    std::vector<int> pids;
    std::vector<int> in_tids;
    int out_tid = -1;
    virtual void on_finalize(Graph& g) {}
    virtual void on_prepare(Graph& g) {}
    virtual void on_resolve_aliases(Graph& g) {}
    virtual bool partial_batch_ok() const { return true; }
    virtual void set_batch_groups(int groups) {}
    virtual bool set_mask(Graph& g, const float* host, size_t n) { return false; }
    virtual size_t mask_floats(Graph& g, int B) { return 0; }
    virtual void reseed(unsigned long long seed) {}
    virtual bool mc_active() const { return false; }
    const char* kind = "op";
    virtual std::string describe_fusion(Graph& g) { return ""; }
    virtual int alias_output() const { return -1; }
    virtual bool reads_tensor(int t) const { return false; }
};

struct Graph {
    std::vector<GTensor> tensors;
    std::vector<GParam> params;
    std::vector<std::unique_ptr<GOp>> ops;
    std::vector<int> inputs, outputs;
    std::vector<GOp*> dropout_ops;
    size_t n_params = 0;
    float* W = nullptr;
    float* G = nullptr;
    float* Wt = nullptr;
    size_t wt_floats = 0;
    bool own_arena = true;
    int maxB = 0;
    bool finalized = false;
    float* workspace = nullptr;
    size_t workspace_bytes = 0;
    hipStream_t aux_stream = nullptr;
    float* aux_workspace = nullptr;
    hipEvent_t ev_fork = nullptr, ev_join = nullptr;
    bool aux_used = false;
    void fork_aux();
    void join_aux();
    hipStream_t stream = nullptr;
    std::vector<float*> allocations;
    struct WtJob { size_t src_off; bool src_in_wt; size_t dst_off; int KK, Cin, Cout; };
    std::vector<WtJob> wt_jobs;
    void* wt_jobs_dev = nullptr;
    int wt_job_blocks = 0;
    bool wt_fresh = false;
    void add_wt_job(size_t src_off, bool src_in_wt, size_t dst_off, int KK, int Cin, int Cout) {
        wt_jobs.push_back({src_off, src_in_wt, dst_off, KK, Cin, Cout});
    }
    void refresh_dgrad_weights();
    struct GradBucket { size_t off = 0, n = 0; int p_lo = 0, p_hi = 0; int ready_op = -1; };
    std::vector<GradBucket> buckets;
    void (*grad_ready)(void* ctx, float* grads, size_t n, hipStream_t stream, hipStream_t aux) = nullptr;
    void* grad_ready_ctx = nullptr;
    void plan_buckets(size_t target_bytes);
    std::vector<char> op_shared, t_boundary;
    int shared_groups = 1;
    bool plan_shared(const std::vector<int>& dup_inputs);

    ~Graph();
// ... 69 lines not shown
```

dl4ds_amd/csrc/graph.hip:

```cpp
#include "graph.h"
#include <cstdlib>
#include "prof.h"
#include "conv_cache.h"
#include <algorithm>
#include <cstring>
#include <cmath>
#include <limits>

static void plan_concat_aliases(Graph& g);
static void plan_grad_aliases(Graph& g);

Graph::~Graph() {
    if (W) derived_filters_release(W, W + n_params);
    if (Wt) derived_filters_release(Wt, Wt + wt_floats);
    for (float* p : allocations) (void)hipFree(p);
    if (own_arena) {
        if (W) (void)hipFree(W);
        if (G) (void)hipFree(G);
    }
    if (Wt) (void)hipFree(Wt);
    if (wt_jobs_dev) (void)hipFree(wt_jobs_dev);
    if (workspace) (void)hipFree(workspace);
    if (aux_workspace) (void)hipFree(aux_workspace);
    if (ev_fork) (void)hipEventDestroy(ev_fork);
// ... 157 lines not shown
        if (op->out_tid < 0) return fail();
        bool all = true, any = false;
        for (int t : op->in_tids) {
            if (t < 0) continue;
            any = true;
            all = all && tdup[t];
        }
        if (!(all && any)) continue;
        const std::string k = op->kind;
        const bool plain = k == "conv2d" || k == "add" || k == "act" || k == "concat" || k == "maxpool2" || k == "pad" || k == "slice";
        if (!plain || !op->partial_batch_ok()) return fail();
        op_shared[i] = 1;
        tdup[op->out_tid] = 1;
        any_shared = true;
    }
    if (!any_shared) return fail();
    for (int o : outputs) if (tdup[o]) return fail();
    for (size_t i = 0; i < ops.size(); ++i) {
        if (op_shared[i]) continue;
        for (int t : ops[i]->in_tids)
            if (t >= 0 && tdup[t] && !tensors[t].is_input) t_boundary[t] = 1;
    }
    for (size_t i = 0; i < ops.size(); ++i) {
        if (!op_shared[i]) continue;
        for (int t : ops[i]->in_tids)
            if (t >= 0 && t_boundary[t]) return fail();
    }
    return true;
}

void Graph::forward(int B, bool training) {
    prepare(B);
    wt_fresh = false;
    GraphPassGuard graph_pass(0);
    derived_filters_invalidate(W, W + n_params);
    if (Wt) derived_filters_invalidate(Wt, Wt + wt_floats);
    derived_filters_refresh(stream, W, W + n_params, 0);
    const bool sh = shared_groups > 1 && !op_shared.empty() && B % shared_groups == 0;
    for (size_t i = 0; i < ops.size(); ++i) {
        GOp* op = ops[i].get();
        if (sh && op_shared[i]) {
            const int Bh = B / shared_groups;
            op->forward(*this, Bh, training);
            if (t_boundary[op->out_tid])
                for (int gi = 1; gi < shared_groups; ++gi)
                    view_axpy(stream, view(op->out_tid, B, false, 0, Bh), view(op->out_tid, B, false, gi * Bh, Bh), 1.f, 0);
        } else {
            op->forward(*this, B, training);
        }
    }
}

void Graph::refresh_dgrad_weights() {
    if (wt_fresh || wt_jobs.empty()) { wt_fresh = true; return; }
    if (wt_jobs_dev == nullptr) {
        std::vector<DgradWeightsJob> host;
        int blocks = 0;
        for (const WtJob& j : wt_jobs) {
            DgradWeightsJob d;
            d.src = (j.src_in_wt ? Wt : W) + j.src_off;
            d.dst = Wt + j.dst_off;
            d.KK = j.KK; d.Cin = j.Cin; d.Cout = j.Cout; d.block0 = blocks;
            blocks += dgrad_weights_job_blocks(j.KK, j.Cin, j.Cout);
            host.push_back(d);
        }
        HIP_CHECK(hipMalloc(&wt_jobs_dev, host.size() * sizeof(DgradWeightsJob)));
        HIP_CHECK(hipMemcpyAsync(wt_jobs_dev, host.data(), host.size() * sizeof(DgradWeightsJob), hipMemcpyHostToDevice, stream));
        HIP_CHECK(hipStreamSynchronize(stream));
        wt_job_blocks = blocks;
    }
    conv2d_dgrad_weights_batched(stream, static_cast<const DgradWeightsJob*>(wt_jobs_dev), (int)wt_jobs.size(), wt_job_blocks);
    wt_fresh = true;
    derived_filters_refresh(stream, Wt, Wt + wt_floats, 1);
}

void Graph::zero_grad_flags() {
    for (auto& t : tensors) t.grad_written = false;
    for (auto& p : params) p.grad_written = false;
}

void Graph::backward(const BwdCtx& c) {
    GraphPassGuard graph_pass(1);
    refresh_dgrad_weights();
    for (auto& t : tensors) { t.grad_written = false; t.pending_add = nullptr; }
    for (int o : outputs) tensors[o].grad_written = true;
    const bool bucketed = c.param_grads && grad_ready != nullptr && !buckets.empty();
    std::vector<char> sent(bucketed ? buckets.size() : 0, 0);
    auto flush_ready = [&](int done_op) {
        for (size_t k = 0; k < buckets.size(); ++k) {
            if (sent[k] || buckets[k].ready_op < done_op) continue;
            for (int pid = buckets[k].p_lo; pid < buckets[k].p_hi; ++pid)
                if (!params[pid].grad_written) { fill(stream, G + params[pid].offset, params[pid].n, 0.f); params[pid].grad_written = true; }
            grad_ready(grad_ready_ctx, G + buckets[k].off, buckets[k].n, stream, (aux_stream && aux_used) ? aux_stream : nullptr);
            sent[k] = 1;
        }
    };
    const bool sh = shared_groups > 1 && !op_shared.empty() && c.B % shared_groups == 0;
    const bool whole = c.b_off == 0 && (c.b_cnt < 0 || c.b_cnt == c.B);
    for (int i = (int)ops.size() - 1; i >= 0; --i) {
        if (sh && op_shared[i]) {
            if (whole && c.param_grads) {
                const int t = ops[i]->out_tid, Bh = c.B / shared_groups;
                if (t_boundary[t] && tensors[t].grad_written)
                    for (int gi = 1; gi < shared_groups; ++gi)
                        view_axpy(stream, view(t, c.B, true, gi * Bh, Bh), view(t, c.B, true, 0, Bh), 1.f, 1);
                BwdCtx ch = c;
                ch.b_off = 0; ch.b_cnt = Bh;
                ops[i]->backward(*this, ch);
            }
        } else {
            ops[i]->backward(*this, c);
        }
        if (bucketed) flush_ready(i);
    }
    join_aux();
    if (bucketed) flush_ready(-1);
    if (c.param_grads) {
        for (auto& p : params)
            if (!p.grad_written) { fill(stream, G + p.offset, p.n, 0.f); p.grad_written = true; }
    }
}

namespace {

struct AttFusion {
    bool fuse_pool = false, fuse_scale = false, fuse_dx = false;
    float* pool = nullptr;
    int pool_tiles = 0;
    float* scale = nullptr;
    float* dmean = nullptr;
    float* ds = nullptr;
    bool ds_ready = false;
    int att_in = -1, att_out = -1;
};

static bool defer_ok(Graph& g, int tid);

struct ConvOp : GOp {
    int in, w, b, add, out, KS, Cout, relu, d2s;
    size_t wt_off = 0;
    bool add_grad_shared = false;
    AttFusion* att_after = nullptr;
    AttFusion* att_before = nullptr;
    ConvOp() { kind = "conv2d"; }
    TView in_view(Graph& g, int B, int bo, int bc) {
        if (att_before && att_before->fuse_scale) {
            TView v = g.view(att_before->att_in, B, false, bo, bc);
            const GTensor& t = g.tensors[in];
            v.sc = att_before->scale + (size_t)bo * t.nmul * t.C;
            return v;
        }
        return g.view(in, B, false, bo, bc);
    }
    TView dy_view(Graph& g, int B, int bo, int bc) {
        if (att_after && att_after->fuse_dx) {
            DL4DS_REQUIRE(d2s <= 1 && bo == 0 && (bc < 0 || bc == B), "fused attention backward: whole batches, no depth_to_space");
            TView v = g.view(att_after->att_out, B, true, bo, bc);
            v.sc = att_after->scale;
            v.sh = att_after->dmean;
            return v;
        }
        return out_view(g, true, B, bo, bc);
    }
    void on_prepare(Graph& g) override {
        if (add_grad_shared) g.tensors[add].grad = g.tensors[out].grad;
        plan_two_adds(g);
        if (add_grad_inplace) g.tensors[add].grad = g.tensors[out].grad;
    }
    void on_resolve_aliases(Graph& g) override {
        if (add >= 0 && (add_grad_shared || add_grad_inplace)) g.tensors[add].grad = g.tensors[out].grad;
    }
    bool add_grad_inplace = false;
    void plan_two_adds(Graph& g) {
        add_grad_inplace = false;
        if (add < 0 || add_grad_shared || d2s > 1 || g.aux_stream || att_before || att_after || test_env("DL4DS_NO_TWO_ADD_INPLACE")) return;
        GTensor& r = g.tensors[add];
        for (int o : g.outputs) if (o == add) return;
        if (r.is_input || !r.requires_grad || r.grad_masked || r.galias || r.alias_of >= 0 || r.n_conv_in != 1 || r.n_add_in != 0 ||
            r.n_masking != 0 || r.n_other != 2 || r.n_fused_add != 2 || r.per_sample() != g.tensors[out].per_sample())
            return;
        int me = -1, other = -1, consumer = -1;
        for (int i = 0; i < (int)g.ops.size(); ++i) {
            ConvOp* c = dynamic_cast<ConvOp*>(g.ops[i].get());
            if (!c) continue;
            if (c == this) me = i;
            else if (c->add == add) other = i;
            if (c->in == add) { if (c->att_before || c->att_after) return; consumer = i; }
        }
        if (me < 0 || other < 0 || consumer < 0) return;
        ConvOp* oc = static_cast<ConvOp*>(g.ops[other].get());
        if (oc->d2s > 1 || oc->add_grad_shared || oc->att_before || oc->att_after || g.tensors[oc->out].per_sample() != r.per_sample()) return;
        if (g.tensors[out].galias || g.tensors[out].alias_of >= 0) return;
        if (!(consumer < me && me < other)) return;
        add_grad_inplace = true;
        r.two_add_inplace = true;
    }
    void on_finalize(Graph& g) override {
        if (add >= 0 && d2s <= 1 && !exp_env("DL4DS_NO_GRAD_SHARE")) {
            const GTensor& r = g.tensors[add];
            bool is_output = false;
            for (int o : g.outputs) is_output |= (o == add);
            add_grad_shared = !r.is_input && !is_output && r.requires_grad && r.n_conv_in == 0 && r.n_add_in == 0 &&
                              r.n_masking == 0 && r.n_other == 1 && r.per_sample() == g.tensors[out].per_sample();
        }
        if (add >= 0 && !add_grad_shared && !exp_env("DL4DS_NO_MASK_FUSION")) {
            GTensor& r = g.tensors[add];
            bool is_output = false;
            for (int o : g.outputs) is_output |= (o == add);
            if (r.relu_out && !r.is_input && !is_output && r.n_other == r.n_fused_add) r.grad_masked = true;
        }
        wt_off = g.reserve_wt(g.params[w].n);
        g.add_wt_job(g.params[w].offset, false, wt_off, KS * KS, g.tensors[in].C, Cout);
        GTensor& t = g.tensors[out];
        bool is_output = false;
        for (int o : g.outputs) is_output |= (o == out);
        t.grad_masked = relu && !is_output && (t.n_conv_in + t.n_add_in + t.n_masking) >= 1 && t.n_other == 0 &&
                        !exp_env("DL4DS_NO_MASK_FUSION");
    }
    TView out_view(Graph& g, bool grad, int B, int bo, int bc) {
        const GTensor& ti = g.tensors[in];
        const GTensor& to = g.tensors[out];
        float* base = (grad ? to.grad : to.data) + (size_t)bo * to.per_sample();
        const int N = (bc < 0 ? B : bc) * to.nmul;
        if (d2s > 1) return make_view_d2s(base, N, ti.H, ti.W, Cout, d2s);
        if ((!grad || to.galias) && to.alias_of >= 0) return g.view(out, B, grad, bo, bc);
        return make_view(base, N, ti.H, ti.W, Cout);
    }
    void forward(Graph& g, int B, bool) override {
        ConvEpilogue ep;
        ep.bias = (b >= 0) ? g.wp(b) : nullptr;
        if (add >= 0) ep.add = g.view(add, B, false);
        ep.relu = relu;
        if (att_after && att_after->fuse_pool) ep.pool = att_after->pool;
        conv2d_forward(g.stream, in_view(g, B, 0, -1), g.wp(w), KS, out_view(g, false, B, 0, -1), ep);
    }
    size_t workspace_bytes(Graph& g, int B) override {
        TView x = g.view(in, B, false);
        TView dz = make_view(nullptr, x.N, x.H, x.W, Cout);
        const size_t att_ws = (size_t)(1024 + x.N) * ((size_t)KS * KS * x.C * Cout + Cout) * sizeof(float);
        return std::max(std::max(conv2d_wgrad_workspace_bytes(x, dz, KS), bias_grad_workspace_bytes(dz)), att_before ? att_ws : 0);
    }
    void backward(Graph& g, const BwdCtx& c) override {
        if (!g.tensors[out].grad_written) return;
        TView dY = dy_view(g, c.B, c.b_off, c.b_cnt);
        if (relu && !g.tensors[out].grad_masked) {
            DL4DS_REQUIRE(!dY.sc, "fused attention backward needs a linear producer");
            bias_act_backward(g.stream, dY, out_view(g, false, c.B, c.b_off, c.b_cnt), dY, nullptr, 0, g.workspace,
                              g.workspace_bytes);
        }
        if (add >= 0 && wants_grad(g, add, c)) {
            GTensor& ra = g.tensors[add];
            bool defer = !add_grad_shared && !ra.grad_written && ra.n_conv_in == 1 && ra.n_add_in == 0 && ra.n_masking == 0 &&
                         ra.n_other == 1 && ra.n_fused_add == 1 && d2s <= 1 && !dY.sc && defer_ok(g, add) &&
                         !exp_env("DL4DS_NO_DEFERRED_ADD");
            const bool inplace_here = add_grad_inplace && ra.two_add_inplace && !dY.sc;
            if (ra.two_add_inplace && !add_grad_inplace && !ra.grad_written && !ra.pending_add && d2s <= 1 && !dY.sc && defer_ok(g, add))
                defer = true;
            if (exp_env("DL4DS_ADD_DEBUG"))
                fprintf(stderr, "conv add grad: op out=%d add=%d defer=%d shared=%d written=%d n_conv_in=%d n_add_in=%d n_masking=%d n_other=%d n_fused_add=%d d2s=%d masked=%d C=%d H=%d B=%d\n",
                        out, add, (int)defer, (int)add_grad_shared, (int)ra.grad_written, ra.n_conv_in, ra.n_add_in, ra.n_masking, ra.n_other,
                        ra.n_fused_add, d2s, (int)ra.grad_masked, ra.C, ra.H, c.B);
            if (defer) {
                ra.pending_add = dY.p;
                ra.pending_view = dY;
            } else if (inplace_here && !ra.grad_written && dY.p == g.view(add, c.B, true, c.b_off, c.b_cnt).p) {
            } else if (!add_grad_shared || inplace_here) {
                if (g.tensors[add].grad_masked)
                    view_axpy_masked(g.stream, dY, g.view(add, c.B, false, c.b_off, c.b_cnt), g.view(add, c.B, true, c.b_off, c.b_cnt),
                                     g.tensors[add].grad_written);
                else
                    view_axpy(g.stream, dY, g.view(add, c.B, true, c.b_off, c.b_cnt), 1.f, g.tensors[add].grad_written);
            }
            if (!defer) g.tensors[add].grad_written = true;
        }
        if (c.param_grads) {
            const bool need_db = b >= 0;
            g.fork_aux();
            const bool on_aux = aux_enabled(g);
            hipStream_t ws_stream = on_aux ? g.aux_stream : g.stream;
            float* ws_buf = on_aux ? g.aux_workspace : g.workspace;
            bool done = false;
            if (att_before && att_before->fuse_scale && c.b_off == 0 && (c.b_cnt < 0 || c.b_cnt == c.B) &&
                !exp_env("DL4DS_NO_DS_FUSION")) {
                done = conv2d_direct_wgrad_attention(g.stream, g.view(att_before->att_in, c.B, false), dY, KS, att_before->scale,
                                                     g.wp(w), g.gp(w), g.params[w].grad_written, need_db ? g.gp(b) : nullptr,
                                                     need_db ? (int)g.params[b].grad_written : 0, att_before->ds, g.workspace,
                                                     g.workspace_bytes);
                att_before->ds_ready = done;
            }
            if (!done)
                conv2d_wgrad(ws_stream, in_view(g, c.B, c.b_off, c.b_cnt), dY, KS, g.gp(w),
                             g.params[w].grad_written, need_db ? g.gp(b) : nullptr,
                             need_db ? (int)g.params[b].grad_written : 0, ws_buf, g.workspace_bytes);
            g.params[w].grad_written = true;
            if (need_db) g.params[b].grad_written = true;
        }
        if (wants_grad(g, in, c)) {
            float* wt = g.Wt + wt_off;
            ConvEpilogue ep;
            ep.accumulate = g.tensors[in].grad_written;
            if (g.tensors[in].grad_masked) ep.mask = g.view(in, c.B, false, c.b_off, c.b_cnt);
            if (g.tensors[in].pending_add) {
                ep.add = g.tensors[in].pending_view;
                g.tensors[in].pending_add = nullptr;
            }
            conv2d_forward(g.stream, dY, wt, KS, g.view(in, c.B, true, c.b_off, c.b_cnt), ep);
            g.tensors[in].grad_written = true;
        }
    }
};

static bool defer_ok(Graph& g, int tid) {
    for (auto& up : g.ops)
        if (ConvOp* c = dynamic_cast<ConvOp*>(up.get()))
            if (c->in == tid) return !c->att_before && !c->att_after;
    return false;
}

struct ChAttOp : GOp {
    int in, out, w1, b1, w2, b2, Cr, T5;
    AttFusion fz;
    ConvOp* producer = nullptr;
    ConvOp* consumer = nullptr;
    ChAttOp() { kind = "chatt"; }
    AttShape shape(Graph& g, int B) {
        const GTensor& t = g.tensors[in];
        AttShape s;
        if (T5 > 0) { s.G = B; s.R = t.nmul * t.H; s.P = t.W; }
        else { s.G = B * t.nmul; s.R = t.H * t.W; s.P = 1; }
        s.C = t.C; s.Cr = Cr;
        return s;
    }
    int pool_tiles(Graph& g) { const GTensor& t = g.tensors[in]; return conv2d_narrow_pair_tiles_per_image(t.H, t.W); }
    size_t saved_floats_per_sample(Graph& g) override {
        const GTensor& t = g.tensors[in];
        const size_t inst = (T5 > 0) ? (size_t)t.W : (size_t)t.nmul;
        return inst * (4 * (size_t)t.C + Cr) + (T5 > 0 ? 0 : (size_t)t.nmul * pool_tiles(g) * 8 + 16);
    }
    size_t workspace_bytes(Graph& g, int B) override { return chatt_workspace_bytes(shape(g, B)); }
    void ptrs(Graph& g, int, float*& mean, float*& hidden, float*& scale, float*& dmean, float*& pool, float** ds_out = nullptr) {
        AttShape s = shape(g, g.maxB);
        const size_t inst = (size_t)s.G * s.P;
        mean = saved; scale = mean + inst * s.C; hidden = scale + inst * s.C; dmean = hidden + inst * s.Cr;
        float* dsp = dmean + inst * s.C;
        if (ds_out) *ds_out = dsp;
        pool = dsp + ((inst * s.C + 3) & ~(size_t)3);
    }
    void on_finalize(Graph& g) override {
        for (auto& op : g.ops) {
            ConvOp* c = dynamic_cast<ConvOp*>(op.get());
            if (!c) continue;
            if (c->out == in) producer = c;
            if (c->in == out) consumer = c;
        }
        fz.att_in = in; fz.att_out = out;
        if (producer) producer->att_after = &fz;
        if (consumer) consumer->att_before = &fz;
    }
    void on_prepare(Graph& g) override {
        fz.fuse_pool = fz.fuse_scale = fz.fuse_dx = false;
        if (T5 > 0 || test_env("DL4DS_NO_TAIL_FUSION")) return;
        const int B = g.maxB;
        float *mean, *hidden, *scale, *dmean, *pool;
        ptrs(g, B, mean, hidden, scale, dmean, pool, &fz.ds);
        fz.scale = scale; fz.dmean = dmean; fz.pool = pool; fz.pool_tiles = pool_tiles(g);
        const GTensor& ti = g.tensors[in];
        const GTensor& to = g.tensors[out];
        auto is_output = [&](int t) { for (int o : g.outputs) if (o == t) return true; return false; };
        const bool in_private = !is_output(in) && ti.n_conv_in == 0 && ti.n_add_in == 0 && ti.n_masking == 0 && ti.n_other == 1;
        if (producer && producer->d2s <= 1 && ti.C <= 8) {
            ConvEpilogue ep;
            ep.bias = producer->b >= 0 ? g.wp(producer->b) : nullptr;
            if (producer->add >= 0) ep.add = g.view(producer->add, B, false);
            TView pin = producer->in_view(g, B, 0, -1), pout = g.view(in, B, false);
            fz.fuse_pool = !conv2d_direct_eligible(pin, pout, producer->KS) && conv2d_narrow_pair_ok(pin, pout, producer->KS, ep);
        }
        if (consumer && !is_output(out) && to.n_conv_in == 1 && to.n_add_in == 0 && to.n_masking == 0 && to.n_other == 0 && consumer->KS == 3) {
            TView x = g.view(in, B, false);
            x.sc = scale;
            TView y = make_view(nullptr, x.N, x.H, x.W, consumer->Cout);
            fz.fuse_scale = conv2d_direct_eligible(x, y, 3);
        }
        if (producer && in_private && producer->relu == 0 && producer->add < 0 && producer->d2s <= 1 && producer->KS == 3 &&
            !ti.grad_masked) {
            TView dz = g.view(out, B, true);
            dz.sc = scale; dz.sh = dmean;
            TView px = producer->in_view(g, B, 0, -1);
            TView dz_plain = dz;
            dz_plain.sc = dz_plain.sh = nullptr;
// ... 47 lines not shown
    int out;
    ConcatOp() { kind = "concat"; }
    TView slice(Graph& g, int B, bool grad, int k, int bo, int bc) {
        TView v = g.view(out, B, grad, bo, bc);
        int off = 0;
        for (int i = 0; i < k; ++i) off += g.tensors[ins[i]].C;
        v.p += off;
        v.C = g.tensors[ins[k]].C;
        v.vec = v.vec && ((off & 3) == 0) && ((v.C & 3) == 0);
        return v;
    }
    void forward(Graph& g, int B, bool) override {
        {
            const TView wide = g.view(out, B, false);
            ConcatSlice sl[4];
            int n = 0, off = 0;
            bool ok = wide.d2s <= 1 && wide.ld == wide.C && wide.nstride == (size_t)wide.H * wide.W * wide.C && !exp_env("DL4DS_NO_CONCAT_JOIN");
            for (size_t k = 0; k < ins.size() && ok; ++k) {
                const GTensor& ti = g.tensors[ins[k]];
                if (ti.alias_parent != out) {
                    const TView d = g.view(ins[k], B, false);
                    ok = n < 4 && d.d2s <= 1 && d.ld == d.C && d.nstride == (size_t)d.H * d.W * d.C && !d.sc;
                    if (ok) sl[n++] = ConcatSlice{d.p, nullptr, off, ti.C, 0};
                }
                off += ti.C;
            }
            if (ok && n >= 2) {
                concat_join(g.stream, wide.p, wide.ld, (size_t)wide.N * wide.H * wide.W, sl, n);
                return;
            }
        }
        for (size_t k = 0; k < ins.size(); ++k) {
            if (g.tensors[ins[k]].alias_parent == out) continue;
            view_axpy(g.stream, g.view(ins[k], B, false), slice(g, B, false, (int)k, 0, -1), 1.f, 0);
        }
    }
    void backward(Graph& g, const BwdCtx& c) override {
        if (!g.tensors[out].grad_written) return;
        {
            const TView wide = g.view(out, c.B, true, c.b_off, c.b_cnt);
            const bool wide_plain = wide.d2s <= 1 && wide.ld == wide.C && wide.nstride == (size_t)wide.H * wide.W * wide.C;
            ConcatSlice sl[4];
            int n = 0, off = 0;
            bool ok = wide_plain && !exp_env("DL4DS_NO_CONCAT_SPLIT");
            for (size_t k = 0; k < ins.size() && ok; ++k)
                for (size_t j = 0; j < k; ++j) ok = ok && ins[j] != ins[k];
            for (size_t k = 0; k < ins.size() && ok; ++k) {
                const GTensor& ti = g.tensors[ins[k]];
                if (wants_grad(g, ins[k], c) && !ti.galias) {
                    const TView d = g.view(ins[k], c.B, true, c.b_off, c.b_cnt);
                    ok = n < 4 && d.d2s <= 1 && d.ld == d.C && d.nstride == (size_t)d.H * d.W * d.C;
                    const float* mk = nullptr;
                    if (ok && ti.grad_masked) {
                        const TView m = g.view(ins[k], c.B, false, c.b_off, c.b_cnt);
                        ok = m.d2s <= 1 && m.ld == m.C && m.nstride == (size_t)m.H * m.W * m.C && !m.sc;
                        mk = m.p;
                    }
                    if (ok) sl[n++] = ConcatSlice{d.p, mk, off, ti.C, ti.grad_written ? 1 : 0};
                }
                off += ti.C;
            }
            if (ok && n >= 2) {
                concat_split(g.stream, wide.p, wide.ld, (size_t)wide.N * wide.H * wide.W, sl, n);
                for (size_t k = 0; k < ins.size(); ++k)
                    if (wants_grad(g, ins[k], c)) g.tensors[ins[k]].grad_written = true;
                return;
            }
        }
        for (size_t k = 0; k < ins.size(); ++k) {
            if (!wants_grad(g, ins[k], c)) continue;
            if (g.tensors[ins[k]].galias) { g.tensors[ins[k]].grad_written = true; continue; }
            TView mask{nullptr, 0, 0, 0, 0, 0, 0, 0};
            if (g.tensors[ins[k]].grad_masked) mask = g.view(ins[k], c.B, false, c.b_off, c.b_cnt);
            view_axpy_masked(g.stream, slice(g, c.B, true, (int)k, c.b_off, c.b_cnt), mask,
                             g.view(ins[k], c.B, true, c.b_off, c.b_cnt), g.tensors[ins[k]].grad_written);
            g.tensors[ins[k]].grad_written = true;
        }
    }
};

struct AddOp : GOp {
    int a, b, out, relu;
    AddOp() { kind = "add"; }
    void forward(Graph& g, int B, bool) override {
        add_act(g.stream, g.tensors[a].data, g.tensors[b].data, g.tensors[out].data,
                g.tensors[out].per_sample() * B, relu);
    }
    void backward(Graph& g, const BwdCtx& c) override {
        if (!g.tensors[out].grad_written) return;
        TView dY = g.view(out, c.B, true, c.b_off, c.b_cnt);
        if (relu) {
            TView none{nullptr, 0, 0, 0, 0, 0, 0, 0};
            bias_act_backward(g.stream, dY, g.view(out, c.B, false, c.b_off, c.b_cnt), dY, nullptr, 0, g.workspace,
                              g.workspace_bytes);
        }
        if (a != b && wants_grad(g, a, c) && wants_grad(g, b, c) && g.tensors[a].grad_masked && g.tensors[b].grad_masked &&
            !exp_env("DL4DS_NO_MASKED_PAIR")) {
            const size_t ps = g.tensors[a].per_sample();
            const size_t off = (size_t)c.b_off * ps, n = (size_t)(c.b_cnt < 0 ? c.B : c.b_cnt) * ps;
            if (g.tensors[b].per_sample() == ps &&
                masked_axpy_pair(g.stream, g.tensors[out].grad + off, g.tensors[a].data + off, g.tensors[a].grad + off, g.tensors[a].grad_written,
                                 g.tensors[b].data + off, g.tensors[b].grad + off, g.tensors[b].grad_written, n)) {
                g.tensors[a].grad_written = true;
                g.tensors[b].grad_written = true;
                return;
            }
        }
        for (int t : {a, b}) {
            if (!wants_grad(g, t, c)) continue;
            if (exp_env("DL4DS_ADD_DEBUG"))
                fprintf(stderr, "add op grad: out=%d operand=%d masked=%d written=%d C=%d H=%d B=%d\n", out, t, (int)g.tensors[t].grad_masked,
                        (int)g.tensors[t].grad_written, g.tensors[t].C, g.tensors[t].H, c.B);
            if (g.tensors[t].grad_masked) {
                const size_t ps = g.tensors[t].per_sample();
                const size_t off = (size_t)c.b_off * ps, n = (size_t)(c.b_cnt < 0 ? c.B : c.b_cnt) * ps;
                masked_axpy(g.stream, g.tensors[out].grad + off, g.tensors[t].data + off, g.tensors[t].grad + off, n,
                            g.tensors[t].grad_written);
            } else {
                view_axpy(g.stream, dY, g.view(t, c.B, true, c.b_off, c.b_cnt), 1.f, g.tensors[t].grad_written);
            }
            g.tensors[t].grad_written = true;
        }
    }
};

struct ActOp : GOp {
    int in, out, act;
    ActOp() { kind = "act"; }
    void forward(Graph& g, int B, bool) override {
        act_forward(g.stream, g.tensors[in].data, g.tensors[out].data, g.tensors[out].per_sample() * B, act);
    }
    void backward(Graph& g, const BwdCtx& c) override {
        if (!g.tensors[out].grad_written || !wants_grad(g, in, c)) return;
        const size_t ps = g.tensors[in].per_sample();
        const size_t off = (size_t)c.b_off * ps;
        const size_t n = (size_t)(c.b_cnt < 0 ? c.B : c.b_cnt) * ps;
        act_backward(g.stream, g.tensors[in].data + off, g.tensors[out].grad + off, g.tensors[in].grad + off, n, act,
                     g.tensors[in].grad_written);
        g.tensors[in].grad_written = true;
    }
};

struct MaxPoolOp : GOp {
    int in, out;
    MaxPoolOp() { kind = "maxpool2"; }
    void forward(Graph& g, int B, bool) override {
        maxpool2_forward(g.stream, g.view(in, B, false), g.view(out, B, false));
    }
    void backward(Graph& g, const BwdCtx& c) override {
        if (!g.tensors[out].grad_written || !wants_grad(g, in, c)) return;
        const GTensor& t = g.tensors[in];
        TView dx = g.view(in, c.B, true, c.b_off, c.b_cnt);
        int acc = t.grad_written;
        if (!acc && ((t.H | t.W) & 1)) {
            fill(g.stream, dx.p, (size_t)dx.N * dx.H * dx.W * dx.C, 0.f);
            acc = 1;
        }
        maxpool2_backward(g.stream, g.view(in, c.B, false, c.b_off, c.b_cnt), g.view(out, c.B, false, c.b_off, c.b_cnt),
                          g.view(out, c.B, true, c.b_off, c.b_cnt), dx, acc, t.grad_masked ? 1 : 0);
        g.tensors[in].grad_written = true;
    }
};

static void bilinear_axis_tables(int in_size, int out_size, std::vector<int>& idx, std::vector<float>& w) {
    const float scale = (float)in_size / (float)out_size;
    idx.assign((size_t)out_size * 2, 0);
    w.assign((size_t)out_size * 2, 0.f);
    for (int o = 0; o < out_size; ++o) {
        const float src = ((float)o + 0.5f) * scale - 0.5f;
        const float fl = std::floor(src);
        const float f = src - fl;
        idx[(size_t)o * 2] = std::max((int)fl, 0);
// ... 429 lines not shown
```

dl4ds_amd/csrc/ops.h:

```cpp
#pragma once
#include "common.h"

struct ConvEpilogue {
    const float* bias = nullptr;
    TView add{nullptr, 0, 0, 0, 0, 0, 0, 0};
    TView mask{nullptr, 0, 0, 0, 0, 0, 0, 0};
    int relu = 0;
    int accumulate = 0;
    float* pool = nullptr;
};
void conv2d_forward(hipStream_t s, const TView& in, const float* w, int KS, const TView& out,
                    const ConvEpilogue& ep);
void conv2d_dgrad_weights(hipStream_t s, const float* w, float* wt, int KS, int Cin, int Cout);
struct DgradWeightsJob { const float* src; float* dst; int KK, Cin, Cout, block0; };
int dgrad_weights_job_blocks(int KK, int Cin, int Cout);
void conv2d_dgrad_weights_batched(hipStream_t s, const DgradWeightsJob* jobs_dev, int nj, int blocks);
size_t conv2d_wgrad_workspace_bytes(const TView& x, const TView& dz, int KS);
void conv2d_wgrad(hipStream_t s, const TView& x, const TView& dz, int KS, float* dw, int accumulate, float* db,
                  int accumulate_db, float* workspace, size_t workspace_bytes);
bool conv2d_direct_forward(hipStream_t s, const TView& in, const float* w, int KS, const TView& out,
                           const ConvEpilogue& ep);
bool conv2d_narrow_forward(hipStream_t s, const TView& in, const float* w, int KS, const TView& out,
                           const ConvEpilogue& ep);
bool conv2d_point_forward(hipStream_t s, const TView& in, const float* w, int KS, const TView& out, const ConvEpilogue& ep);
bool conv2d_narrow_pair_ok(const TView& in, const TView& out, int KS, const ConvEpilogue& ep);
int conv2d_narrow_pair_tiles_per_image(int H, int W);
bool conv2d_direct_eligible(const TView& in, const TView& out, int KS);
bool conv2d_direct_wgrad_attention(hipStream_t s, const TView& x_raw, const TView& dz, int KS, const float* scale, const float* w,
                                   float* dw, int accumulate, float* db, int accumulate_db, float* ds, float* workspace,
                                   size_t workspace_bytes);
int conv2d_narrow_wgrad_slabs(const TView& x, const TView& dz, int KS);
int conv2d_narrow_wgrad(hipStream_t s, const TView& x, const TView& dz, int KS, float* partial, int max_slabs);
bool conv2d_gemm_forward(hipStream_t s, const TView& in, const float* w, int KS, const TView& out, const ConvEpilogue& ep, int max_hw);
bool conv2d_wino_forward(hipStream_t s, const TView& in, const float* w, const TView& out, const ConvEpilogue& ep);
bool conv2d_split_forward(hipStream_t s, const TView& in, const float* w, const TView& out, const ConvEpilogue& ep);
void derived_filters_invalidate(const float* lo, const float* hi);
void derived_filters_refresh(hipStream_t s, const float* lo, const float* hi, int kind);
void derived_filters_release(const float* lo, const float* hi);
void split_filters_invalidate(const float* lo, const float* hi);
void split_filters_refresh(hipStream_t s, const float* lo, const float* hi, int kind);
void split_filters_release(const float* lo, const float* hi);
bool conv2d_wino_wgrad(hipStream_t s, const TView& x, const TView& dy, float* dw, int accumulate, float* db, int accumulate_db);
bool conv2d_stream_forward(hipStream_t s, const TView& in, const float* w, int KS, const TView& out,
                           const ConvEpilogue& ep);
int conv2d_direct_wgrad_slabs(const TView& x, const TView& dz, int KS);
int conv2d_direct_wgrad(hipStream_t s, const TView& x, const TView& dz, int KS, float* partial, int slabs);
void conv2d_transpose_forward(hipStream_t s, const TView& in, const float* w, int KS, int stride,
                              const TView& out, int relu, float* workspace, size_t workspace_bytes);
void conv2d_transpose_dgrad(hipStream_t s, const TView& dz, const float* w, int KS, int stride,
                            const TView& dx, int accumulate, float* workspace, size_t workspace_bytes,
                            const TView* relu_mask = nullptr);
void conv2d_transpose_wgrad(hipStream_t s, const TView& x, const TView& dz, int KS, int stride,
                            float* dw, int accumulate, float* workspace, size_t workspace_bytes);
size_t conv2d_transpose_workspace_bytes(const TView& in, const TView& out, int KS, int stride);

size_t bias_grad_workspace_bytes(const TView& dy);
void bias_act_backward(hipStream_t s, const TView& dy, const TView& y, const TView& dz, float* db,
                       int accumulate_db, float* workspace, size_t workspace_bytes);
void view_axpy(hipStream_t s, const TView& src, const TView& dst, float alpha, int accumulate);
void view_axpy_masked(hipStream_t s, const TView& src, const TView& mask, const TView& dst, int accumulate);
struct ConcatSlice { float* dst; const float* mask; int off, C, accumulate; };
void concat_split(hipStream_t s, const float* src, int ld, size_t npx, const ConcatSlice* slices, int n);
void concat_join(hipStream_t s, float* dst, int ld, size_t npx, const ConcatSlice* slices, int n);
void masked_axpy(hipStream_t s, const float* dy, const float* y, float* dst, size_t n, int accumulate);
bool masked_axpy_pair(hipStream_t s, const float* dy, const float* ya, float* da, int acc_a, const float* yb, float* db, int acc_b, size_t n);
void add_act(hipStream_t s, const float* a, const float* b, float* out, size_t n, int relu);
enum ActKind { ACT_NONE = 0, ACT_RELU = 1, ACT_SIGMOID = 2, ACT_TANH = 3, ACT_ELU = 4,
               ACT_LEAKY_RELU = 5, ACT_SELU = 6, ACT_GELU = 7 };
void act_forward(hipStream_t s, const float* x, float* y, size_t n, int kind);
void act_backward(hipStream_t s, const float* x, const float* dy, float* dx, size_t n, int kind,
                  int accumulate);
void fill(hipStream_t s, float* p, size_t n, float v);
void dwconv_forward(hipStream_t s, const float* x, const float* k, const float* bias, float* y, int N, int H, int W, int C,
                    int KS, int flip, int accumulate);
size_t dwconv_wgrad_workspace_bytes(int C, int KS);
void dwconv_wgrad(hipStream_t s, const float* x, const float* dy, float* dk, float* db, int accumulate, int N, int H, int W, int C,
                  int KS, float* ws, size_t ws_bytes);
size_t metrics_workspace_bytes(int N, int H, int W, int C);
void image_metrics(hipStream_t s, const float* y_true, const float* y_pred, int N, int H, int W, int C, float* pair_out_dev,
                   float* grid_out_dev, float* range_out_dev, float* workspace, size_t workspace_bytes);
size_t spearman_workspace_bytes(size_t S, size_t L);
void spearman(hipStream_t s, const float* a, const float* b, size_t S, size_t L, size_t seg_stride, size_t elem_stride, double* out,
              void* workspace, size_t workspace_bytes);
enum ScalerOp { SCALER_OP_NONE = 0, SCALER_OP_MUL = 1, SCALER_OP_ADD = 2, SCALER_OP_SUB = 3, SCALER_OP_DIV = 4 };
enum ScalerNan { SCALER_NAN_FILL = 0, SCALER_NAN_MASK = 1 };
size_t scaler_cells(const size_t* shape, int ndim, const int* reduce);
size_t scaler_stats_workspace_bytes(const size_t* shape, int ndim, const int* reduce, int is_double);
void scaler_stats(hipStream_t s, const void* x, int is_double, const size_t* shape, int ndim, const int* reduce, double* out,
                  unsigned* nan_flag, unsigned* mask_bits, void* workspace, size_t workspace_bytes);
void scaler_apply(hipStream_t s, const void* x, void* out, int is_double, const size_t* shape, int ndim, const int* reduce, int op1,
                  const void* a, int op2, const void* b, int nan_mode, double fill, const unsigned* mask_bits);
constexpr int ENS_MAX_MEMBERS = 256, ENS_MAX_QUANTILES = 32;
void ensemble_reduce(hipStream_t s, const float* members, size_t K, size_t n, size_t member_stride, const float* q_host, int nq,
                     float* mean, float* std_, float* mn, float* mx, float* quant);
size_t ensemble_score_workspace_bytes(size_t n, size_t B);
void ensemble_score(hipStream_t s, const float* members, size_t K, size_t n, size_t member_stride, const float* obs, size_t B,
                    unsigned long long elem_offset, const float* scale, int fair, unsigned long long seed, const float* q_host, int nq,
                    float* crps, float* sqerr, float* var, int* rank, double* sample_out, double* cell_acc,
                    unsigned long long* rank_hist, unsigned long long* covered, void* workspace, size_t workspace_bytes);
constexpr int EXC_MAX_THRESHOLDS = 16;
size_t exc_walk_limit(size_t K);
void ensemble_exceedance(hipStream_t s, const float* members, size_t K, size_t n, size_t member_stride, const float* obs, size_t B,
                         const float* thr, int T, int thr_per_cell, short* count, long long* sample_out, long long* cell_acc,
                         unsigned long long* table);
size_t fss_workspace_bytes(int N, int H, int W, int C, int T);
void fss_check_args(int N, int H, int W, int C, const float* thresholds, int T, const int* windows, int S);
void fss(hipStream_t s, const float* y, const float* p, int N, int H, int W, int C, const float* thresholds, int T,
         const int* windows, int S, long long* sums, long long* cont, long long* valid, void* workspace, size_t workspace_bytes);
size_t distribution_workspace_bytes(size_t S, size_t L, size_t seg_stride, size_t elem_stride);
void distribution_check_args(size_t S, size_t L, const double* q, int Q, const float* edges, int E);
void distribution(hipStream_t s, const float* y, const float* p, size_t S, size_t L, size_t seg_stride, size_t elem_stride,
                  const double* q, int Q, const float* edges, int E, double* quant, double* w1, long long* ks, long long* hist,
                  long long* valid, void* workspace, size_t workspace_bytes);
size_t quantile_table_workspace_bytes(size_t N, size_t per);
void quantile_table(hipStream_t s, const float* x, size_t N, size_t per, const double* q, int Q, float* table, long long* valid,
                    void* workspace, size_t workspace_bytes);
void qmap_apply(hipStream_t s, const float* x, float* out, size_t B, size_t per, const float* model_tab, const float* obs_tab,
                const float* target_tab, int Q, int kind, int keep_unfitted, unsigned long long* counts);
// ... 77 lines not shown
```

dl4ds_amd/ops.py:

```python
import ctypes
import numpy as np
from . import _lib
from .device import DeviceArray

LOSS_KINDS = {'mae': 0, 'mse': 1, 'dssim': 2, 'dssim_mae': 3, 'dssim_mse': 4, 'dssim_mae_mse': 5,
              'msdssim': 6, 'msdssim_mae': 7, 'msdssim_mae_mse': 8}


def _d(a):
    return None if a is None else DeviceArray.from_numpy(np.asarray(a, np.float32))


def _p(d):
    return None if d is None else d.ptr


def conv2d(x, w, b=None, add=None, relu=False, d2s=0):
    n, h, wd, cin = x.shape
    ks, _, ci, cout = w.shape
    assert ci == cin
    dx, dw, db, da = _d(x), _d(w), _d(b), _d(add)
    if d2s > 1:
        y = DeviceArray.zeros((n, h * d2s, wd * d2s, cout // (d2s * d2s)))
    else:
        y = DeviceArray.zeros((n, h, wd, cout))
    _lib.check(_lib.lib().dl4ds_op_conv2d_fwd(dx.ptr, dw.ptr, _p(db), _p(da), y.ptr, n, h, wd, cin, cout, ks,
                                              int(relu), int(d2s)))
    return y.numpy()


def conv2d_epilogue(x, w, b=None, add=None, mask=None, relu=False, accumulate_into=None):
    n, h, wd, cin = x.shape
    ks, _, ci, cout = w.shape
    assert ci == cin
    dx, dw, db, da, dm = _d(x), _d(w), _d(b), _d(add), _d(mask)
    y = DeviceArray.zeros((n, h, wd, cout)) if accumulate_into is None else _d(accumulate_into)
    _lib.check(_lib.lib().dl4ds_op_conv2d_epilogue(dx.ptr, dw.ptr, _p(db), _p(da), _p(dm), y.ptr, n, h, wd, cin, cout, ks,
                                                   int(relu), int(accumulate_into is not None)))
    return y.numpy()


def conv2d_dgrad(dz, w, d2s=0, accumulate_into=None):
    ks, _, cin, cout = w.shape
    if d2s > 1:
        n, h, wd = dz.shape[0], dz.shape[1] // d2s, dz.shape[2] // d2s
    else:
        n, h, wd = dz.shape[:3]
    ddz, dw = _d(dz), _d(w)
    dx = DeviceArray.zeros((n, h, wd, cin)) if accumulate_into is None else _d(accumulate_into)
    _lib.check(_lib.lib().dl4ds_op_conv2d_dgrad(ddz.ptr, dw.ptr, dx.ptr, n, h, wd, cin, cout, ks, int(d2s),
                                                int(accumulate_into is not None)))
    return dx.numpy()


def conv2d_wgrad(x, dz, ks, d2s=0, accumulate_into=None):
    n, h, wd, cin = x.shape
    cout = dz.shape[-1] * (d2s * d2s if d2s > 1 else 1)
    dx, ddz = _d(x), _d(dz)
    dw = DeviceArray.zeros((ks, ks, cin, cout)) if accumulate_into is None else _d(accumulate_into)
    _lib.check(_lib.lib().dl4ds_op_conv2d_wgrad(dx.ptr, ddz.ptr, dw.ptr, n, h, wd, cin, cout, ks, int(d2s),
                                                int(accumulate_into is not None)))
    return dw.numpy()


def bias_act_bwd(dy, y=None, want_db=True):
    n, h, w, c = dy.shape
    ddy, dyy = _d(dy), _d(y)
    db = DeviceArray.zeros((c,)) if want_db else None
    _lib.check(_lib.lib().dl4ds_op_bias_act_bwd(ddy.ptr, _p(dyy), _p(db), n, h, w, c))
    return ddy.numpy(), (db.numpy() if want_db else None)


def conv2d_transpose(x, w, stride, relu=False):
    n, h, wd, cin = x.shape
    ks, _, cout, ci = w.shape
    assert ci == cin
    dx, dw = _d(x), _d(w)
    y = DeviceArray.zeros((n, h * stride, wd * stride, cout))
    _lib.check(_lib.lib().dl4ds_op_conv2d_transpose_fwd(dx.ptr, dw.ptr, y.ptr, n, h, wd, cin, cout, ks, stride, int(relu)))
    return y.numpy()


def conv2d_transpose_dgrad(dz, w, stride):
    ks, _, cout, cin = w.shape
    n, h, wd = dz.shape[0], dz.shape[1] // stride, dz.shape[2] // stride
    ddz, dw = _d(dz), _d(w)
    dx = DeviceArray.zeros((n, h, wd, cin))
    _lib.check(_lib.lib().dl4ds_op_conv2d_transpose_dgrad(ddz.ptr, dw.ptr, dx.ptr, n, h, wd, cin, cout, ks, stride, 0))
    return dx.numpy()


def conv2d_transpose_wgrad(x, dz, ks, stride):
    n, h, wd, cin = x.shape
    cout = dz.shape[-1]
    dx, ddz = _d(x), _d(dz)
    dw = DeviceArray.zeros((ks, ks, cout, cin))
    _lib.check(_lib.lib().dl4ds_op_conv2d_transpose_wgrad(dx.ptr, ddz.ptr, dw.ptr, n, h, wd, cin, cout, ks, stride, 0))
    return dw.numpy()


def depth_to_space(x, r):
    n, h, w, c = x.shape
    dx = _d(x)
    y = DeviceArray.zeros((n, h * r, w * r, c // (r * r)))
    _lib.check(_lib.lib().dl4ds_op_depth_to_space(dx.ptr, y.ptr, n, h, w, c, r))
    return y.numpy()


def space_to_depth(y, r):
    n, hh, ww, cp = y.shape
    h, w, c = hh // r, ww // r, cp * r * r
    dy = _d(y)
    x = DeviceArray.zeros((n, h, w, c))
    _lib.check(_lib.lib().dl4ds_op_space_to_depth(dy.ptr, x.ptr, n, h, w, c, r))
    return x.numpy()


def maxpool2(x):
    n, h, w, c = x.shape
    dx = _d(x)
    y = DeviceArray.zeros((n, h // 2, w // 2, c))
    _lib.check(_lib.lib().dl4ds_op_maxpool2_fwd(dx.ptr, y.ptr, n, h, w, c))
# ... 155 lines not shown
```

include/dl4ds_hip.h:

```cpp
#ifndef DL4DS_HIP_H
#define DL4DS_HIP_H
#include <stddef.h>
#include <stdint.h>

#ifdef __cplusplus
extern "C" {
#endif

typedef struct dl4ds_graph dl4ds_graph;
typedef struct dl4ds_trainer dl4ds_trainer;

const char* dl4ds_last_error(void);
int dl4ds_init(int device);
int dl4ds_device_count(int* n);
int dl4ds_device_name(char* buf, int buflen);
int dl4ds_malloc(void** p_dev, size_t bytes);
int dl4ds_free(void* p_dev);
int dl4ds_memcpy_h2d(void* dst_dev, const void* src_host, size_t bytes);
int dl4ds_memcpy_d2h(void* dst_host, const void* src_dev, size_t bytes);
int dl4ds_memcpy_d2d(void* dst_dev, const void* src_dev, size_t bytes);
int dl4ds_host_register(void* p_host, size_t bytes);
int dl4ds_host_unregister(void* p_host);
int dl4ds_memset(void* p_dev, int value, size_t bytes);
int dl4ds_sync(void);
int dl4ds_debug_raise_device_error(int code);
int dl4ds_event_timer_start(void);
int dl4ds_event_timer_stop(float* ms);
int dl4ds_profile_enable(int on);
int dl4ds_profile_filter(const char* tag_prefix);
int dl4ds_profile_report(char* json_buf, size_t buflen);


int dl4ds_op_conv2d_fwd(const float* x_dev, const float* w_dev, const float* b_dev, const float* add_dev,
                        float* y_dev, int N, int H, int W, int Cin, int Cout, int KS, int relu, int d2s_r);
int dl4ds_op_conv2d_epilogue(const float* x_dev, const float* w_dev, const float* b_dev, const float* add_dev,
                             const float* mask_dev, float* y_dev, int N, int H, int W, int Cin, int Cout, int KS, int relu,
                             int accumulate);
int dl4ds_op_conv2d_dgrad(const float* dz_dev, const float* w_dev, float* dx_dev, int N, int H, int W,
                          int Cin, int Cout, int KS, int d2s_r, int accumulate);
int dl4ds_op_conv2d_wgrad(const float* x_dev, const float* dz_dev, float* dw_dev, int N, int H, int W,
                          int Cin, int Cout, int KS, int d2s_r, int accumulate);
int dl4ds_op_bias_act_bwd(float* dy_dev, const float* y_dev, float* db_dev, int N, int H, int W, int C);
int dl4ds_op_conv2d_transpose_fwd(const float* x_dev, const float* w_dev, float* y_dev, int N, int H, int W,
                                  int Cin, int Cout, int KS, int stride, int relu);
int dl4ds_op_conv2d_transpose_dgrad(const float* dz_dev, const float* w_dev, float* dx_dev, int N, int H,
                                    int W, int Cin, int Cout, int KS, int stride, int accumulate);
int dl4ds_op_conv2d_transpose_wgrad(const float* x_dev, const float* dz_dev, float* dw_dev, int N, int H,
                                    int W, int Cin, int Cout, int KS, int stride, int accumulate);
int dl4ds_op_depth_to_space(const float* x_dev, float* y_dev, int N, int H, int W, int C, int r);
int dl4ds_op_space_to_depth(const float* y_dev, float* x_dev, int N, int H, int W, int C, int r);
int dl4ds_op_maxpool2_fwd(const float* x_dev, float* y_dev, int N, int H, int W, int C);
int dl4ds_op_maxpool2_bwd(const float* x_dev, const float* y_dev, const float* dy_dev, float* dx_dev, int N,
                          int H, int W, int C);
int dl4ds_op_dwconv_fwd(const float* x_dev, const float* k_dev, const float* bias_dev, float* y_dev, int N, int H, int W, int C,
                        int KS);
int dl4ds_op_dwconv_bwd(const float* x_dev, const float* k_dev, const float* dy_dev, float* dx_dev, float* dk_dev, float* db_dev,
                        int N, int H, int W, int C, int KS, int accumulate);
int dl4ds_op_layernorm_fwd(const float* x_dev, const float* gamma_dev, const float* beta_dev, float* y_dev, size_t npix, int C,
                           float eps, int relu);
int dl4ds_op_layernorm_bwd(const float* x_dev, const float* y_dev, const float* dy_dev, const float* gamma_dev, float* dx_dev,
                           float* dgamma_dev, float* dbeta_dev, size_t npix, int C, float eps, int relu, int accumulate);
int dl4ds_op_batchnorm_fwd(const float* x_dev, const float* gamma_dev, const float* beta_dev, float* moving_mean_dev,
                           float* moving_var_dev, float* y_dev, float* saved_dev, size_t npix, int C, float eps,
                           float momentum, int training, int relu);
int dl4ds_op_batchnorm_bwd(const float* x_dev, const float* y_dev, const float* dy_dev, const float* gamma_dev,
                           const float* saved_dev, float* dx_dev, float* dgamma_dev, float* dbeta_dev, size_t npix, int C,
                           int relu, int accumulate);
int dl4ds_op_resize_bilinear_fwd(const float* x_dev, float* y_dev, int N, int H, int W, int C, int Ho, int Wo);
int dl4ds_op_resize_bilinear_bwd(const float* dy_dev, float* dx_dev, int N, int H, int W, int C, int Ho, int Wo);
int dl4ds_op_localconv_fwd(const float* x_dev, const float* w_dev, const float* b_dev, float* y_dev, int N,
                           int H, int W, int C, int F);
int dl4ds_op_localconv_bwd(const float* x_dev, const float* w_dev, const float* dy_dev, float* dx_dev,
                           float* dw_dev, float* db_dev, int N, int H, int W, int C, int F);
int dl4ds_op_chatt_fwd(const float* x_dev, float* y_dev, int G, int R, int P, int C, int Cr, const float* w1_dev,
                       const float* b1_dev, const float* w2_dev, const float* b2_dev, float* saved_dev);
int dl4ds_op_chatt_bwd(const float* x_dev, const float* dy_dev, float* dx_dev, int G, int R, int P, int C, int Cr,
                       const float* w1_dev, const float* w2_dev, const float* saved_dev, float* dw1_dev,
                       float* db1_dev, float* dw2_dev, float* db2_dev);
int dl4ds_op_loss(int kind, const float* y_true_dev, const float* y_pred_dev, float* dpred_dev, int N, int H,
                  int W, int C, float* loss_dev);
int dl4ds_metrics(const float* y_true_dev, const float* y_pred_dev, int N, int H, int W, int C, float* pair_out_dev,
                  float* grid_out_dev, float* range_out_dev);
int dl4ds_spearman(const float* a_dev, const float* b_dev, size_t S, size_t L, size_t seg_stride, size_t elem_stride,
                   double* out_dev);
int dl4ds_scaler_cells(const size_t* shape, int ndim, const int* reduce, size_t* cells_out);
int dl4ds_scaler_stats_workspace_bytes(const size_t* shape, int ndim, const int* reduce, int is_double, size_t* bytes_out);
int dl4ds_scaler_stats(const void* x_dev, int is_double, const size_t* shape, int ndim, const int* reduce, double* out_dev,
                       unsigned* nan_flag_dev, unsigned* mask_bits_dev);
int dl4ds_scaler_apply(const void* x_dev, void* out_dev, int is_double, const size_t* shape, int ndim, const int* reduce, int op1,
                       const void* a_dev, int op2, const void* b_dev, int nan_mode, double fill, const unsigned* mask_bits_dev);
int dl4ds_ensemble_reduce(const float* members_dev, size_t K, size_t n, size_t member_stride, const float* q_host, int nq,
                          float* mean_dev, float* std_dev, float* min_dev, float* max_dev, float* quant_dev);
int dl4ds_ensemble_score(const float* members_dev, size_t K, size_t n, size_t member_stride, const float* obs_dev, size_t B,
                         unsigned long long elem_offset, const float* scale_dev, int fair, unsigned long long seed,
                         const float* q_host, int nq, float* crps_dev, float* sqerr_dev, float* var_dev, int* rank_dev,
                         double* sample_out_dev, double* cell_acc_dev, unsigned long long* rank_hist_dev,
                         unsigned long long* covered_dev);
int dl4ds_ensemble_exceedance(const float* members_dev, size_t K, size_t n, size_t member_stride, const float* obs_dev, size_t B,
                              const float* thr_dev, int T, int thr_per_cell, short* count_dev, long long* sample_out_dev,
                              long long* cell_acc_dev, unsigned long long* table_dev);
int dl4ds_ensemble_exceedance_walk_limit(size_t K, size_t* samples_out);
int dl4ds_fss(const float* y_dev, const float* p_dev, int N, int H, int W, int C, const float* thresholds_host, int T,
              const int* windows_host, int S, long long* sums_dev, long long* cont_dev, long long* valid_dev);
int dl4ds_distribution(const float* y_dev, const float* p_dev, size_t S, size_t L, size_t seg_stride, size_t elem_stride,
                       const double* q_host, int Q, const float* edges_host, int E, double* quant_dev, double* w1_dev,
                       long long* ks_dev, long long* hist_dev, long long* valid_dev);
int dl4ds_quantile_table(const float* x_dev, size_t N, size_t per, const double* q_host, int Q, float* table_dev,
                         long long* valid_dev);
int dl4ds_qmap_apply(const float* x_dev, float* out_dev, size_t B, size_t per, const float* model_tab_dev, const float* obs_tab_dev,
                     const float* target_tab_dev, int Q, int kind, int keep_unfitted, unsigned long long* counts_dev);
int dl4ds_climate_indices(const float* x_dev, size_t N, size_t per, const long long* period_starts_host, int P,
                          const float* thr_dev, int T, int thr_per_cell, int op, int window, int* valid_dev, int* event_dev,
                          float* ext_dev, double* sum_dev);
int dl4ds_spectrum(const float* y_dev, const float* p_dev, int N, int H, int W, int C, int detrend, int window,
                   const int* bin_host, int B, double* power_dev, long long* valid_dev, double* mean_dev);
int dl4ds_op_bce(const float* p_dev, float label, int n, float* loss_dev, float* dp_dev);
int dl4ds_op_adam(float* w_dev, const float* g_dev, float* m_dev, float* v_dev, size_t n, int t, float lr,
                  float beta1, float beta2, float eps, float grad_scale);

int dl4ds_graph_create(dl4ds_graph** g);
// ... 112 lines not shown
```

Before: 5193 HR samples/s.

## Fuse long-skip add into producing conv epilogue and dual-mask backward output

Adds a second-output epilogue to the split and Winograd 3x3 conv kernels. In forward, the conv feeding a long-skip add also writes the skip sum, so the separate add kernel is no longer needed. In backward, a dual-mask form emits the gradients for both add inputs from the consumer conv's dgrad. The aim is to remove the extra elementwise passes over full-resolution activations and gradients, at the cost of new kernel template instantiations, extra stores in the epilogue, and planning logic spread across the graph ops.

```diff
diff --git a/dl4ds_amd/csrc/capi.cpp b/dl4ds_amd/csrc/capi.cpp
--- a/dl4ds_amd/csrc/capi.cpp
+++ b/dl4ds_amd/csrc/capi.cpp
@@ -275,6 +275,34 @@
     ep.relu = relu;
     ep.accumulate = accumulate;
     conv2d_forward(S(), make_view(nc(x), N, H, W, Cin), w, KS, make_view(y, N, H, W, Cout), ep);
+    API_END
+}
+int dl4ds_op_conv2d_second_output(const float* x, const float* w, const float* b, const float* sum_add, float* sum_out, const float* mask,
+                                  const float* mask2, float* y2, float* partial, float* y, int N, int H, int W, int Cin, int Cout, int KS,
+                                  int relu, int* launched) {
+    API_BEGIN
+    DL4DS_REQUIRE(launched != nullptr, "conv2d_second_output: launched is null");
+    ConvEpilogue ep;
+    ep.bias = b;
+    ep.relu = relu;
+    if (sum_add) ep.sum_add = make_view(nc(sum_add), N, H, W, Cout);
+    if (sum_out) ep.sum_out = make_view(sum_out, N, H, W, Cout);
+    if (mask) ep.mask = make_view(nc(mask), N, H, W, Cout);
+    if (mask2) ep.mask2 = make_view(nc(mask2), N, H, W, Cout);
+    if (y2) ep.out2 = make_view(y2, N, H, W, Cout);
+    if (partial) ep.partial = make_view(partial, N, H, W, Cout);
+    *launched = conv2d_forward_fused(S(), make_view(nc(x), N, H, W, Cin), w, KS, make_view(y, N, H, W, Cout), ep) ? 1 : 0;
+    API_END
+}
+int dl4ds_op_add_act(const float* a, const float* b, float* out, size_t n, int relu) {
+    API_BEGIN
+    add_act(S(), a, b, out, n, relu);
+    API_END
+}
+int dl4ds_op_masked_axpy_pair(const float* dy, const float* ya, float* da, const float* yb, float* db, size_t n, int* launched) {
+    API_BEGIN
+    DL4DS_REQUIRE(launched != nullptr, "masked_axpy_pair: launched is null");
+    *launched = masked_axpy_pair(S(), dy, ya, da, 0, yb, db, 0, n) ? 1 : 0;
     API_END
 }
 int dl4ds_op_conv2d_dgrad(const float* dz, const float* w, float* dx, int N, int H, int W, int Cin, int Cout, int KS,
diff --git a/dl4ds_amd/csrc/conv.hip b/dl4ds_amd/csrc/conv.hip
--- a/dl4ds_amd/csrc/conv.hip
+++ b/dl4ds_amd/csrc/conv.hip
@@ -1402,6 +1402,7 @@
 void conv2d_forward(hipStream_t s, const TView& in, const float* w, int KS, const TView& out,
                     const ConvEpilogue& ep) {
     DL4DS_REQUIRE(in.N == out.N && in.H == out.H && in.W == out.W, "conv2d: stride-1 SAME shapes differ");
+    DL4DS_REQUIRE(!ep.sum_out.p && !ep.out2.p, "conv2d: a second output pair goes through conv2d_forward_fused");
     if (conv2d_direct_forward(s, in, w, KS, out, ep)) return;
     if (!exp_env("DL4DS_NO_NARROW") && conv2d_narrow_forward(s, in, w, KS, out, ep)) return;
     DL4DS_REQUIRE(!in.sc && !ep.pool, "conv2d: channel-affine input / pooling partials are only implemented by the direct "
@@ -1427,6 +1428,16 @@
         case 7: dispatch_fwd<7>(s, p, in.N); break;
         default: throw Dl4dsError("conv2d: kernel size " + std::to_string(KS) + " not supported (1,3,5,7)");
     }
+}
+
+bool conv2d_forward_fused(hipStream_t s, const TView& in, const float* w, int KS, const TView& out, const ConvEpilogue& ep) {
+    DL4DS_REQUIRE(in.N == out.N && in.H == out.H && in.W == out.W, "conv2d: stride-1 SAME shapes differ");
+    DL4DS_REQUIRE((ep.sum_out.p != nullptr) != (ep.out2.p != nullptr), "conv2d_forward_fused: one second output pair");
+    if (KS != 3 || in.C < 24 || out.C < 24 || in.sc || ep.pool) return false;
+    bool refused = false;
+    if (conv2d_split_forward(s, in, w, out, ep, &refused)) return true;
+    if (refused) return false;
+    return conv2d_wino_forward(s, in, w, out, ep, &refused);
 }
 
 __global__ void __launch_bounds__(256) dgrad_weights_tiled_kernel(const float* __restrict__ w, float* __restrict__ wt, int KK, int Cin,
diff --git a/dl4ds_amd/csrc/conv_split.hip b/dl4ds_amd/csrc/conv_split.hip
--- a/dl4ds_amd/csrc/conv_split.hip
+++ b/dl4ds_amd/csrc/conv_split.hip
@@ -38,6 +38,9 @@
     int nitems;
     int relu, old;
     int final_pass;
+    const float* sum_add;
+    float* sum_out;
+    size_t sum_add_ns, sum_out_ns;
     unsigned long long* trace;
 };
 
@@ -141,7 +144,7 @@
 #define SPLIT_TRACE_START
 #define SPLIT_TRACE_END
 #endif
-template <bool OLD, bool ADD, bool MASK>
+template <bool OLD, bool ADD, bool MASK, bool SUM = false>
 __global__ void __launch_bounds__(NTHREADS) conv_split_kernel(const SplitParams p) {
     extern __shared__ __attribute__((aligned(16))) unsigned char smem[];
     unsigned char* rowbuf = smem;
@@ -198,12 +201,16 @@
                 const_cast<float*>(ADD ? p.add.p + (size_t)n * p.add.nstride : p.out.p), 0, 0x7fffff00, RSRC3);
             const __amdgpu_buffer_rsrc_t rs_mask = __builtin_amdgcn_make_buffer_rsrc(
                 const_cast<float*>(MASK ? p.mask.p + (size_t)n * p.mask.nstride : p.out.p), 0, 0x7fffff00, RSRC3);
-            i32x4 ov = {0, 0, 0, 0}, av = {0, 0, 0, 0}, mv = {0, 0, 0, 0};
+            const __amdgpu_buffer_rsrc_t rs_sadd = __builtin_amdgcn_make_buffer_rsrc(
+                const_cast<float*>(SUM ? p.sum_add + (size_t)n * p.sum_add_ns : p.out.p), 0, 0x7fffff00, RSRC3);
+            const __amdgpu_buffer_rsrc_t rs_sout = __builtin_amdgcn_make_buffer_rsrc(SUM ? p.sum_out + (size_t)n * p.sum_out_ns : p.out.p, 0, 0x7fffff00, RSRC3);
+            i32x4 ov = {0, 0, 0, 0}, av = {0, 0, 0, 0}, mv = {0, 0, 0, 0}, sv = {0, 0, 0, 0};
             auto request = [&](int yo) __attribute__((always_inline)) {
                 const int eoff = (yo >= y_lo && yo < y_hi && ooff != OOB) ? 0 : OOB;
                 if constexpr (OLD) ov = __builtin_amdgcn_raw_buffer_load_b128(rs_out, (eoff | ooff) + (eoff == 0 ? yo * out_ys : 0), 0, 0);
                 if constexpr (ADD) av = __builtin_amdgcn_raw_buffer_load_b128(rs_add, (eoff | aoff) + (eoff == 0 ? yo * add_ys : 0), 0, 0);
                 if constexpr (MASK) mv = __builtin_amdgcn_raw_buffer_load_b128(rs_mask, (eoff | moff) + (eoff == 0 ? yo * mask_ys : 0), 0, 0);
+                if constexpr (SUM) sv = __builtin_amdgcn_raw_buffer_load_b128(rs_sadd, (eoff | ooff) + (eoff == 0 ? yo * out_ys : 0), 0, 0);
             };
             auto finish = [&](int yo, int buf) __attribute__((always_inline)) {
                 const int eoff = (yo >= y_lo && yo < y_hi && ooff != OOB) ? 0 : OOB;
@@ -231,6 +238,13 @@
                 i32x4 vi;
                 __builtin_memcpy(&vi, &v, 16);
                 __builtin_amdgcn_raw_buffer_store_b128(vi, rs_out, (eoff | ooff) + (eoff == 0 ? yo * out_ys : 0), 0, 0);
+                if constexpr (SUM) {
+                    float4 sa;
+                    __builtin_memcpy(&sa, &sv, 16);
+                    const float4 t = make_float4(sa.x + v.x, sa.y + v.y, sa.z + v.z, sa.w + v.w);
+                    __builtin_memcpy(&vi, &t, 16);
+                    __builtin_amdgcn_raw_buffer_store_b128(vi, rs_sout, (eoff | ooff) + (eoff == 0 ? yo * out_ys : 0), 0, 0);
+                }
             };
             f32x4 acc[3][2];
 #pragma unroll
@@ -399,18 +413,19 @@
     SPLIT_TRACE_END;
 }
 
-template <bool OLD, bool ADD, bool MASK>
+template <bool OLD, bool ADD, bool MASK, bool SUM = false>
 void launch_one(hipStream_t s, const SplitParams& p, int grid) {
     static bool once = false;
     if (!once) {
-        HIP_CHECK(hipFuncSetAttribute(reinterpret_cast<const void*>(conv_split_kernel<OLD, ADD, MASK>), hipFuncAttributeMaxDynamicSharedMemorySize,
+        HIP_CHECK(hipFuncSetAttribute(reinterpret_cast<const void*>(conv_split_kernel<OLD, ADD, MASK, SUM>), hipFuncAttributeMaxDynamicSharedMemorySize,
                                       (int)LDS_BYTES));
         once = true;
     }
-    DL4DS_LAUNCH((conv_split_kernel<OLD, ADD, MASK>), dim3(grid), dim3(NTHREADS), LDS_BYTES, s, p);
+    DL4DS_LAUNCH((conv_split_kernel<OLD, ADD, MASK, SUM>), dim3(grid), dim3(NTHREADS), LDS_BYTES, s, p);
     HIP_CHECK(hipGetLastError());
 }
 void launch_form(hipStream_t s, const SplitParams& p, int grid) {
+    if (p.sum_out) { launch_one<false, false, false, true>(s, p, grid); return; }
     const int f = (p.old ? 4 : 0) | (p.add.p ? 2 : 0) | (p.mask.p ? 1 : 0);
     switch (f) {
         case 0: launch_one<false, false, false>(s, p, grid); break;
@@ -461,7 +476,7 @@
         });
 }
 
-bool conv2d_split_forward(hipStream_t s, const TView& in, const float* w, const TView& out, const ConvEpilogue& ep) {
+bool conv2d_split_forward(hipStream_t s, const TView& in, const float* w, const TView& out, const ConvEpilogue& ep, bool* form_refused) {
     const char* force = test_env("DL4DS_SPLIT_FORCE");
     if (getenv("DL4DS_NO_SPLIT")) return false;
     const bool every_shape = getenv("DL4DS_SPLIT") != nullptr || force != nullptr;
@@ -490,10 +505,21 @@
     if (items >= (1l << 24) || (!force && items * p.nchunk < (long)cu_count())) return false;
     p.nitems = (int)items;
     p.relu = ep.relu;
+    p.sum_add = nullptr; p.sum_out = nullptr; p.sum_add_ns = p.sum_out_ns = 0;
+    if (ep.sum_out.p || ep.out2.p) {
+        auto like_out = [&](const TView& v) { return v.p && v.vec && v.N == out.N && v.H == out.H && v.C == out.C && v.ld == out.ld && v.d2s == out.d2s && v.W == out.W && v.cp == out.cp; };
+        if (ep.out2.p || passes > 1 || ep.add.p || ep.mask.p || ep.accumulate || !like_out(ep.sum_add) || !like_out(ep.sum_out) ||
+            span(ep.sum_add) >= (1ull << 31) || span(ep.sum_out) >= (1ull << 31)) {
+            if (form_refused) *form_refused = true;
+            return false;
+        }
+        p.sum_add = ep.sum_add.p; p.sum_out = ep.sum_out.p;
+        p.sum_add_ns = ep.sum_add.nstride; p.sum_out_ns = ep.sum_out.nstride;
+    }
     const double px = (double)in.N * in.H * in.W;
     const double fl = 2.0 * px * 9.0 * in.C * out.C;
     ProfScope ps(s, std::string("conv_split<3,3>") + (test_env("DL4DS_SPLIT_TAG_FORMS") ? std::string("f") + std::to_string((ep.accumulate ? 4 : 0) | (ep.add.p ? 2 : 0) | (ep.mask.p ? 1 : 0)) + "c" + std::to_string(in.C) + "_" + std::to_string(out.C) : std::string()), fl,
-                 4.0 * (px * (in.C + out.C * (1 + (ep.add.p ? 1 : 0) + (ep.mask.p ? 1 : 0) + (ep.accumulate ? 1 : 0))) + 9.0 * in.C * out.C), fl);
+                 4.0 * (px * (in.C + out.C * (1 + (ep.add.p ? 1 : 0) + (ep.mask.p ? 1 : 0) + (ep.accumulate ? 1 : 0) + (ep.sum_out.p ? 2 : 0))) + 9.0 * in.C * out.C), fl);
     const int per_pass = p.nchunk * (NMW + NHW) * 12 * 64;
     bool need_frag = true;
     u32x4* frag = reinterpret_cast<u32x4*>(
diff --git a/dl4ds_amd/csrc/conv_wino.hip b/dl4ds_amd/csrc/conv_wino.hip
--- a/dl4ds_amd/csrc/conv_wino.hip
+++ b/dl4ds_amd/csrc/conv_wino.hip
@@ -199,7 +199,7 @@
     return true;
 }
 
-bool conv2d_wino_forward(hipStream_t s, const TView& in, const float* w, const TView& out, const ConvEpilogue& ep) {
+bool conv2d_wino_forward(hipStream_t s, const TView& in, const float* w, const TView& out, const ConvEpilogue& ep, bool* form_refused) {
     const bool off = getenv("DL4DS_NO_WINOGRAD") != nullptr;
     const char* force = test_env("DL4DS_WINO_FORCE");
     if (off) return false;
@@ -210,6 +210,12 @@
     auto same_layout = [](const TView& u, const TView& v) { return u.ld == v.ld && u.d2s == v.d2s && u.W == v.W && u.cp == v.cp; };
     if (ep.add.p && !same_layout(ep.add, out)) return false;
     if (ep.mask.p && !same_layout(ep.mask, out)) return false;
+    const bool dual = ep.out2.p != nullptr, sum = ep.sum_out.p != nullptr;
+    const bool second = dual || sum;
+    auto like_out = [&](const TView& v) { return v.p && v.vec && v.N == out.N && v.H == out.H && v.C == out.C && same_layout(v, out); };
+    bool second_ok = !(dual && sum) && !(second && (ep.accumulate || out.d2s > 1));
+    if (sum) second_ok = second_ok && like_out(ep.sum_add) && like_out(ep.sum_out) && !ep.add.p && !ep.mask.p;
+    if (dual) second_ok = second_ok && like_out(ep.mask2) && like_out(ep.out2) && ep.mask.p && !ep.add.p && ep.out2.p != out.p;
     auto span = [](const TView& v) { const size_t r = std::max(v.d2s, 1); return (size_t)8 * v.W * r * r * v.ld * 4; };
     if (span(in) >= (1ull << 31) || span(out) >= (1ull << 31)) return false;
     int KQ, cpass;
@@ -220,10 +226,12 @@
     else return false;
     const int passes = cdiv(in.C, cpass);
     if (passes > 1 && ep.accumulate) return false;
-    const int full_epi = (ep.add.p ? WINO_ADD : 0) | (ep.mask.p ? WINO_MASK : 0) | (ep.accumulate ? WINO_OLDA : 0);
-    if (!wino_epi_built(full_epi) || (passes > 1 && !wino_epi_built(full_epi | WINO_OLDF))) return false;
-    if (test_env("DL4DS_WINO_F44") && conv2d_wino4_forward(s, in, w, out, ep, KQ, cpass, force)) return true;
+    const int plain_epi = (ep.add.p ? WINO_ADD : 0) | (ep.mask.p ? WINO_MASK : 0) | (ep.accumulate ? WINO_OLDA : 0);
+    const int full_epi = plain_epi | (dual ? WINO_MASK2 : 0) | (sum ? WINO_SUM : 0);
+    if (!wino_epi_built(plain_epi) || (passes > 1 && !wino_epi_built(plain_epi | WINO_OLDF))) return false;
+    if (!second && test_env("DL4DS_WINO_F44") && conv2d_wino4_forward(s, in, w, out, ep, KQ, cpass, force)) return true;
     const int NT = (cdiv(out.C, 32) * 32 < cdiv(out.C, 48) * 48) ? 2 : 3;
+    auto refuse_form = [&]() { if (form_refused) *form_refused = true; return false; };
     WinoParams wp;
     ConvParams& p = wp.c;
     p.in = in; p.out = out; p.add = ep.add; p.mask = ep.mask;
@@ -244,11 +252,21 @@
     int SX = (SXmax / wp.nchunk) * wp.nchunk;
     if (force && atoi(force) > 0) SX = std::min(SX, atoi(force) * wp.nchunk);
     if (!force && (long)wp.per_xcd * wp.nchunk < 4l * SX) return false;
+    if (second) {
+        if (!second_ok || test_env("DL4DS_WINO_F44") || !wino_epi_built(full_epi | (passes > 1 ? WINO_OLDF : 0), KQ, NT)) return refuse_form();
+        if (dual && passes > 1 && !(like_out(ep.partial) && ep.partial.p != out.p && ep.partial.p != ep.out2.p)) return refuse_form();
+        wp.x2 = dual ? ep.mask2.p : ep.sum_add.p;
+        wp.x2_ns = dual ? ep.mask2.nstride : ep.sum_add.nstride;
+        wp.o2 = dual ? ep.out2.p : ep.sum_out.p;
+        wp.o2_ns = dual ? ep.out2.nstride : ep.sum_out.nstride;
+        wp.old = ep.partial.p;
+        wp.old_ns = ep.partial.nstride;
+    }
     const double px = (double)in.N * in.H * in.W;
     const double issued = 2.0 * (px / 4.0) * 16.0 * (16.0 * KQ * passes) * (16.0 * NT * wp.nchunk) +
                           (px / 4.0) * (32.0 * in.C * wp.nchunk + 24.0 * out.C * passes);
     ProfScope ps(s, "conv_wino<" + std::to_string(KQ) + "," + std::to_string(NT) + ">", issued,
-                 4.0 * (px * (in.C + out.C * (1 + (ep.add.p ? 1 : 0) + (ep.mask.p ? 1 : 0) + (ep.accumulate ? 1 : 0))) + 9.0 * in.C * out.C),
+                 4.0 * (px * (in.C + out.C * (1 + (ep.add.p ? 1 : 0) + (ep.mask.p ? 1 : 0) + (ep.accumulate ? 1 : 0) + (second ? 2 : 0))) + 9.0 * in.C * out.C),
                  2.0 * px * 9.0 * in.C * out.C);
     const size_t per_pass = (size_t)wp.nchunk * 4 * (16 * KQ * NT) * 64;
     const int total = (int)(per_pass * passes);
@@ -266,6 +284,7 @@
         wp.first = ps_ == 0;
         p.relu = last ? ep.relu : 0;
         const int epi = passes == 1 ? full_epi : ((ps_ ? WINO_OLDF : 0) | (last ? full_epi : 0));
+        if (dual && passes > 1) p.out = last ? out : ep.partial;
         if (KQ == 2) {
             if (NT == 2) launch_wino_22(s, wp, SX, epi); else launch_wino_23(s, wp, SX, epi);
         } else {
diff --git a/dl4ds_amd/csrc/conv_wino_kernel.h b/dl4ds_amd/csrc/conv_wino_kernel.h
--- a/dl4ds_amd/csrc/conv_wino_kernel.h
+++ b/dl4ds_amd/csrc/conv_wino_kernel.h
@@ -16,6 +16,10 @@
     int ntg, per_xcd;
     int tgx, tgy;
     unsigned m_tgx, m_tgy;
+    const float* x2 = nullptr;
+    float* o2 = nullptr;
+    const float* old = nullptr;
+    size_t x2_ns = 0, o2_ns = 0, old_ns = 0;
 #ifdef WINO_TRACE
     unsigned long long* trace;
 #endif
@@ -26,8 +30,13 @@
     WINO_ADD = 2,
     WINO_MASK = 4,
     WINO_OLDA = 8,
+    WINO_MASK2 = 16,
+    WINO_SUM = 32,
 };
-inline bool wino_epi_built(int e) { return e == 0 || e == 1 || e == 2 || e == 3 || e == 4 || e == 5 || e == 8 || e == 12; }
+inline bool wino_epi_built(int e, int KQ = 0, int NT = 0) {
+    if (e == 20 || e == 21 || e == 32) return KQ == 3 && NT == 3;
+    return e == 0 || e == 1 || e == 2 || e == 3 || e == 4 || e == 5 || e == 8 || e == 12;
+}
 
 void launch_wino_22(hipStream_t s, WinoParams& wp, int SX, int epi);
 void launch_wino_23(hipStream_t s, WinoParams& wp, int SX, int epi);
@@ -115,6 +124,8 @@
     constexpr int OOB = (int)0xffffff00u;
     constexpr int RSRC3 = 0x00020000;
     constexpr bool OLDF = (EPI & WINO_OLDF) != 0, ADD = (EPI & WINO_ADD) != 0, MASK = (EPI & WINO_MASK) != 0, OLDA = (EPI & WINO_OLDA) != 0;
+    constexpr bool DUAL = (EPI & WINO_MASK2) != 0, SUM = (EPI & WINO_SUM) != 0, X2 = DUAL || SUM;
+    static_assert(!(DUAL && SUM) && (!DUAL || MASK) && !(X2 && OLDA), "second-output forms");
     extern __shared__ __attribute__((aligned(16))) float lds[];
     float* const raw = lds;
     float* const Pb = lds + 2 * GM::RAWS * 4;
@@ -381,11 +392,24 @@
             const size_t pb_ = cur.y0 * osy + cur.x0 * osx;
             const __amdgpu_buffer_rsrc_t ro = __builtin_amdgcn_make_buffer_rsrc(
                 reinterpret_cast<char*>(a.out.p) + ((size_t)cur.n * a.out.nstride + pb_) * 4, 0, 0x7fffff00, RSRC3);
-            i32x4_t e_old[(OLDF || OLDA) ? ND : 1], e_add[ADD ? ND : 1], e_mask[MASK ? ND : 1];
-            if (OLDF || OLDA) {
+            i32x4_t e_old[(OLDF || OLDA) ? ND : 1], e_add[ADD ? ND : 1], e_mask[MASK ? ND : 1], e_x2[X2 ? ND : 1];
+            if (OLDF && DUAL) {
+                const __amdgpu_buffer_rsrc_t rp = __builtin_amdgcn_make_buffer_rsrc(
+                    const_cast<char*>(reinterpret_cast<const char*>(wp.old)) + ((size_t)cur.n * wp.old_ns + pb_) * 4, 0, 0x7fffff00, RSRC3);
+#pragma unroll
+                for (int u = 0; u < ND; ++u) e_old[u] = __builtin_amdgcn_raw_buffer_load_b128(rp, dv[u], 0, 0);
+            } else if (OLDF || OLDA) {
 #pragma unroll
                 for (int u = 0; u < ND; ++u) e_old[u] = __builtin_amdgcn_raw_buffer_load_b128(ro, dv[u], 0, 0);
             }
+            if (X2) {
+                const __amdgpu_buffer_rsrc_t rx = __builtin_amdgcn_make_buffer_rsrc(
+                    const_cast<char*>(reinterpret_cast<const char*>(wp.x2)) + ((size_t)cur.n * wp.x2_ns + pb_) * 4, 0, 0x7fffff00, RSRC3);
+#pragma unroll
+                for (int u = 0; u < ND; ++u) e_x2[u] = __builtin_amdgcn_raw_buffer_load_b128(rx, dv[u], 0, 0);
+            }
+            const __amdgpu_buffer_rsrc_t ro2 = __builtin_amdgcn_make_buffer_rsrc(
+                reinterpret_cast<char*>(X2 ? wp.o2 : a.out.p) + ((size_t)cur.n * (X2 ? wp.o2_ns : a.out.nstride) + pb_) * 4, 0, 0x7fffff00, RSRC3);
             if (ADD) {
                 const __amdgpu_buffer_rsrc_t ra_ = __builtin_amdgcn_make_buffer_rsrc(
                     reinterpret_cast<char*>(a.add.p) + ((size_t)cur.n * a.add.nstride + pb_) * 4, 0, 0x7fffff00, RSRC3);
@@ -409,6 +433,19 @@
                 if (OLDF) r = add4(r, __builtin_bit_cast(f32x4, e_old[u]));
                 if (ADD) r = add4(r, __builtin_bit_cast(f32x4, e_add[u]));
                 r[0] = fmaxf(r[0], floor_v); r[1] = fmaxf(r[1], floor_v); r[2] = fmaxf(r[2], floor_v); r[3] = fmaxf(r[3], floor_v);
+                if (DUAL) {
+                    const f32x4 m = __builtin_bit_cast(f32x4, e_x2[u]);
+                    f32x4 r2;
+                    r2[0] = m[0] > 0.f ? r[0] : 0.f; r2[1] = m[1] > 0.f ? r[1] : 0.f;
+                    r2[2] = m[2] > 0.f ? r[2] : 0.f; r2[3] = m[3] > 0.f ? r[3] : 0.f;
+                    __builtin_amdgcn_raw_buffer_store_b128(__builtin_bit_cast(i32x4_t, r2), ro2, dv[u], 0, 0);
+                }
+                if (SUM) {
+                    const f32x4 sv = __builtin_bit_cast(f32x4, e_x2[u]);
+                    f32x4 r2;
+                    r2[0] = sv[0] + r[0]; r2[1] = sv[1] + r[1]; r2[2] = sv[2] + r[2]; r2[3] = sv[3] + r[3];
+                    __builtin_amdgcn_raw_buffer_store_b128(__builtin_bit_cast(i32x4_t, r2), ro2, dv[u], 0, 0);
+                }
                 if (MASK) {
                     const f32x4 m = __builtin_bit_cast(f32x4, e_mask[u]);
                     r[0] = m[0] > 0.f ? r[0] : 0.f; r[1] = m[1] > 0.f ? r[1] : 0.f;
@@ -498,6 +535,14 @@
         case 5: launch_one<KQ, NT, 5>(s, wp, SX); break;
         case 8: launch_one<KQ, NT, 8>(s, wp, SX); break;
         case 12: launch_one<KQ, NT, 12>(s, wp, SX); break;
+        case 20: case 21: case 32:
+            if constexpr (KQ == 3 && NT == 3) {
+                if (epi == 20) launch_one<KQ, NT, 20>(s, wp, SX);
+                else if (epi == 21) launch_one<KQ, NT, 21>(s, wp, SX);
+                else launch_one<KQ, NT, 32>(s, wp, SX);
+                break;
+            }
+            [[fallthrough]];
         default: throw Dl4dsError("conv_wino: epilogue form " + std::to_string(epi) + " is not built");
     }
 }
diff --git a/dl4ds_amd/csrc/graph.h b/dl4ds_amd/csrc/graph.h
--- a/dl4ds_amd/csrc/graph.h
+++ b/dl4ds_amd/csrc/graph.h
@@ -29,6 +29,7 @@
     int alias_parent = -1;
     bool galias = false;
     bool grad_masked = false;
+    bool add_grads_done = false;
     size_t per_sample() const { return (size_t)nmul * H * W * C; }
 };
 
diff --git a/dl4ds_amd/csrc/graph.hip b/dl4ds_amd/csrc/graph.hip
--- a/dl4ds_amd/csrc/graph.hip
+++ b/dl4ds_amd/csrc/graph.hip
@@ -263,7 +263,7 @@
 void Graph::backward(const BwdCtx& c) {
     GraphPassGuard graph_pass(1);
     refresh_dgrad_weights();
-    for (auto& t : tensors) { t.grad_written = false; t.pending_add = nullptr; }
+    for (auto& t : tensors) { t.grad_written = false; t.pending_add = nullptr; t.add_grads_done = false; }
     for (int o : outputs) tensors[o].grad_written = true;
     const bool bucketed = c.param_grads && grad_ready != nullptr && !buckets.empty();
     std::vector<char> sent(bucketed ? buckets.size() : 0, 0);
@@ -323,6 +323,8 @@
     bool add_grad_shared = false;
     AttFusion* att_after = nullptr;
     AttFusion* att_before = nullptr;
+    int sum_add = -1, sum_out = -1, dual_a = -1, dual_b = -1;
+    static bool long_skip_active(const Graph& g) { return !(g.shared_groups > 1 && !g.op_shared.empty()); }
     ConvOp() { kind = "conv2d"; }
     TView in_view(Graph& g, int B, int bo, int bc) {
         if (att_before && att_before->fuse_scale) {
@@ -408,12 +410,27 @@
         return make_view(base, N, ti.H, ti.W, Cout);
     }
     void forward(Graph& g, int B, bool) override {
+        if (sum_add >= 0 && long_skip_active(g)) return;
+        launch_forward(g, B, false);
+    }
+    bool launch_forward(Graph& g, int B, bool with_sum) {
         ConvEpilogue ep;
         ep.bias = (b >= 0) ? g.wp(b) : nullptr;
         if (add >= 0) ep.add = g.view(add, B, false);
         ep.relu = relu;
         if (att_after && att_after->fuse_pool) ep.pool = att_after->pool;
+        if (with_sum) {
+            ep.sum_add = g.view(sum_add, B, false);
+            ep.sum_out = g.view(sum_out, B, false);
+            return conv2d_forward_fused(g.stream, in_view(g, B, 0, -1), g.wp(w), KS, out_view(g, false, B, 0, -1), ep);
+        }
         conv2d_forward(g.stream, in_view(g, B, 0, -1), g.wp(w), KS, out_view(g, false, B, 0, -1), ep);
+        return true;
+    }
+    bool forward_with_sum(Graph& g, int B) {
+        if (launch_forward(g, B, true)) return true;
+        launch_forward(g, B, false);
+        return false;
     }
     size_t workspace_bytes(Graph& g, int B) override {
         TView x = g.view(in, B, false);
@@ -485,7 +502,26 @@
                 ep.add = g.tensors[in].pending_view;
                 g.tensors[in].pending_add = nullptr;
             }
-            conv2d_forward(g.stream, dY, wt, KS, g.view(in, c.B, true, c.b_off, c.b_cnt), ep);
+            bool done = false;
+            if (dual_a >= 0 && long_skip_active(g) && !ep.accumulate && !ep.mask.p && !ep.add.p && !dY.sc && wants_grad(g, dual_a, c) &&
+                wants_grad(g, dual_b, c)) {
+                GTensor& ta = g.tensors[dual_a];
+                GTensor& tb = g.tensors[dual_b];
+                if (ta.grad_masked && tb.grad_masked && !ta.grad_written && !tb.grad_written) {
+                    ep.mask = g.view(dual_a, c.B, false, c.b_off, c.b_cnt);
+                    ep.mask2 = g.view(dual_b, c.B, false, c.b_off, c.b_cnt);
+                    ep.out2 = g.view(dual_b, c.B, true, c.b_off, c.b_cnt);
+                    ep.partial = g.view(in, c.B, true, c.b_off, c.b_cnt);
+                    done = conv2d_forward_fused(g.stream, dY, wt, KS, g.view(dual_a, c.B, true, c.b_off, c.b_cnt), ep);
+                    if (done) {
+                        ta.grad_written = tb.grad_written = true;
+                        g.tensors[in].add_grads_done = true;
+                    } else {
+                        ep = ConvEpilogue();
+                    }
+                }
+            }
+            if (!done) conv2d_forward(g.stream, dY, wt, KS, g.view(in, c.B, true, c.b_off, c.b_cnt), ep);
             g.tensors[in].grad_written = true;
         }
     }
@@ -699,12 +735,48 @@
 struct AddOp : GOp {
     int a, b, out, relu;
     AddOp() { kind = "add"; }
+    ConvOp* sum_conv = nullptr;
+    void on_prepare(Graph& g) override { plan_long_skip(g); }
+    void plan_long_skip(Graph& g) {
+        sum_conv = nullptr;
+        for (auto& up : g.ops)
+            if (ConvOp* cv = dynamic_cast<ConvOp*>(up.get())) {
+                if (cv->sum_out == out) cv->sum_add = cv->sum_out = -1;
+                if (cv->in == out) cv->dual_a = cv->dual_b = -1;
+            }
+        if (relu || a == b || test_env("DL4DS_NO_LONG_SKIP_FUSION")) return;
+        const GTensor& to = g.tensors[out];
+        if (g.tensors[a].per_sample() != to.per_sample() || g.tensors[b].per_sample() != to.per_sample()) return;
+        auto is_output = [&](int t) { for (int o : g.outputs) if (o == t) return true; return false; };
+        auto dense = [&](int t) { return g.tensors[t].alias_of < 0 && !g.tensors[t].galias; };
+        if (!dense(a) || !dense(b) || !dense(out)) return;
+        for (int t : {b, a}) {
+            const GTensor& tt = g.tensors[t];
+            if (is_output(t) || tt.is_input || tt.n_conv_in || tt.n_other || tt.n_masking || tt.n_add_in != 1) continue;
+            for (auto& up : g.ops) {
+                ConvOp* cv = dynamic_cast<ConvOp*>(up.get());
+                if (!cv || cv->out != t) continue;
+                if (cv->KS == 3 && cv->d2s <= 1 && cv->add < 0 && !cv->att_before && !cv->att_after) {
+                    cv->sum_add = (t == b) ? a : b;
+                    cv->sum_out = out;
+                    sum_conv = cv;
+                }
+            }
+            if (sum_conv) break;
+        }
+        if (!is_output(out) && to.n_conv_in == 1 && to.n_other == 0 && to.n_masking == 0 && to.n_add_in == 0 && to.requires_grad)
+            for (auto& up : g.ops) {
+                ConvOp* cv = dynamic_cast<ConvOp*>(up.get());
+                if (cv && cv->in == out && cv->KS == 3 && !cv->att_before && !cv->att_after) { cv->dual_a = a; cv->dual_b = b; }
+            }
+    }
     void forward(Graph& g, int B, bool) override {
+        if (sum_conv && ConvOp::long_skip_active(g) && sum_conv->forward_with_sum(g, B)) return;
         add_act(g.stream, g.tensors[a].data, g.tensors[b].data, g.tensors[out].data,
                 g.tensors[out].per_sample() * B, relu);
     }
     void backward(Graph& g, const BwdCtx& c) override {
-        if (!g.tensors[out].grad_written) return;
+        if (!g.tensors[out].grad_written || g.tensors[out].add_grads_done) return;
         TView dY = g.view(out, c.B, true, c.b_off, c.b_cnt);
         if (relu) {
             TView none{nullptr, 0, 0, 0, 0, 0, 0, 0};
diff --git a/dl4ds_amd/csrc/ops.h b/dl4ds_amd/csrc/ops.h
--- a/dl4ds_amd/csrc/ops.h
+++ b/dl4ds_amd/csrc/ops.h
@@ -8,9 +8,12 @@
     int relu = 0;
     int accumulate = 0;
     float* pool = nullptr;
+    TView sum_add{nullptr, 0, 0, 0, 0, 0, 0, 0}, sum_out{nullptr, 0, 0, 0, 0, 0, 0, 0};
+    TView mask2{nullptr, 0, 0, 0, 0, 0, 0, 0}, out2{nullptr, 0, 0, 0, 0, 0, 0, 0}, partial{nullptr, 0, 0, 0, 0, 0, 0, 0};
 };
 void conv2d_forward(hipStream_t s, const TView& in, const float* w, int KS, const TView& out,
                     const ConvEpilogue& ep);
+bool conv2d_forward_fused(hipStream_t s, const TView& in, const float* w, int KS, const TView& out, const ConvEpilogue& ep);
 void conv2d_dgrad_weights(hipStream_t s, const float* w, float* wt, int KS, int Cin, int Cout);
 struct DgradWeightsJob { const float* src; float* dst; int KK, Cin, Cout, block0; };
 int dgrad_weights_job_blocks(int KK, int Cin, int Cout);
@@ -32,8 +35,10 @@
 int conv2d_narrow_wgrad_slabs(const TView& x, const TView& dz, int KS);
 int conv2d_narrow_wgrad(hipStream_t s, const TView& x, const TView& dz, int KS, float* partial, int max_slabs);
 bool conv2d_gemm_forward(hipStream_t s, const TView& in, const float* w, int KS, const TView& out, const ConvEpilogue& ep, int max_hw);
-bool conv2d_wino_forward(hipStream_t s, const TView& in, const float* w, const TView& out, const ConvEpilogue& ep);
-bool conv2d_split_forward(hipStream_t s, const TView& in, const float* w, const TView& out, const ConvEpilogue& ep);
+bool conv2d_wino_forward(hipStream_t s, const TView& in, const float* w, const TView& out, const ConvEpilogue& ep,
+                         bool* form_refused = nullptr);
+bool conv2d_split_forward(hipStream_t s, const TView& in, const float* w, const TView& out, const ConvEpilogue& ep,
+                          bool* form_refused = nullptr);
 void derived_filters_invalidate(const float* lo, const float* hi);
 void derived_filters_refresh(hipStream_t s, const float* lo, const float* hi, int kind);
 void derived_filters_release(const float* lo, const float* hi);
diff --git a/dl4ds_amd/ops.py b/dl4ds_amd/ops.py
--- a/dl4ds_amd/ops.py
+++ b/dl4ds_amd/ops.py
@@ -38,6 +38,47 @@
     _lib.check(_lib.lib().dl4ds_op_conv2d_epilogue(dx.ptr, dw.ptr, _p(db), _p(da), _p(dm), y.ptr, n, h, wd, cin, cout, ks,
                                                    int(relu), int(accumulate_into is not None)))
     return y.numpy()
+
+
+def conv2d_sum_output(x, w, b, s, relu=False):
+    n, h, wd, cin = x.shape
+    ks, _, ci, cout = w.shape
+    assert ci == cin and s.shape == (n, h, wd, cout)
+    dx, dw, db, ds = _d(x), _d(w), _d(b), _d(s)
+    y, y2 = DeviceArray.zeros((n, h, wd, cout)), DeviceArray.zeros((n, h, wd, cout))
+    ok = ctypes.c_int(0)
+    _lib.check(_lib.lib().dl4ds_op_conv2d_second_output(dx.ptr, dw.ptr, _p(db), ds.ptr, y2.ptr, None, None, None, None, y.ptr, n, h, wd,
+                                                        cin, cout, ks, int(relu), ctypes.byref(ok)))
+    return y.numpy(), y2.numpy(), bool(ok.value)
+
+
+def conv2d_dual_mask(x, w, mask, mask2):
+    n, h, wd, cin = x.shape
+    ks, _, ci, cout = w.shape
+    assert ci == cin and mask.shape == mask2.shape == (n, h, wd, cout)
+    dx, dw, dm, dm2 = _d(x), _d(w), _d(mask), _d(mask2)
+    y, y2, part = (DeviceArray.zeros((n, h, wd, cout)) for _ in range(3))
+    ok = ctypes.c_int(0)
+    _lib.check(_lib.lib().dl4ds_op_conv2d_second_output(dx.ptr, dw.ptr, None, None, None, dm.ptr, dm2.ptr, y2.ptr, part.ptr, y.ptr, n, h,
+                                                        wd, cin, cout, ks, 0, ctypes.byref(ok)))
+    return y.numpy(), y2.numpy(), bool(ok.value)
+
+
+def add_act(a, b, relu=False):
+    da, db = _d(a), _d(b)
+    out = DeviceArray.zeros(a.shape)
+    _lib.check(_lib.lib().dl4ds_op_add_act(da.ptr, db.ptr, out.ptr, a.size, int(relu)))
+    return out.numpy()
+
+
+def masked_axpy_pair(dy, ya, yb):
+    ddy, dya, dyb = _d(dy), _d(ya), _d(yb)
+    da, db = DeviceArray.zeros(dy.shape), DeviceArray.zeros(dy.shape)
+    ok = ctypes.c_int(0)
+    _lib.check(_lib.lib().dl4ds_op_masked_axpy_pair(ddy.ptr, dya.ptr, da.ptr, dyb.ptr, db.ptr, dy.size, ctypes.byref(ok)))
+    if not ok.value:
+        raise ValueError('masked_axpy_pair: size not a multiple of four')
+    return da.numpy(), db.numpy()
 
 
 def conv2d_dgrad(dz, w, d2s=0, accumulate_into=None):
diff --git a/include/dl4ds_hip.h b/include/dl4ds_hip.h
--- a/include/dl4ds_hip.h
+++ b/include/dl4ds_hip.h
@@ -36,6 +36,13 @@
 int dl4ds_op_conv2d_epilogue(const float* x_dev, const float* w_dev, const float* b_dev, const float* add_dev,
                              const float* mask_dev, float* y_dev, int N, int H, int W, int Cin, int Cout, int KS, int relu,
                              int accumulate);
+int dl4ds_op_conv2d_second_output(const float* x_dev, const float* w_dev, const float* b_dev, const float* sum_add_dev,
+                                  float* sum_out_dev, const float* mask_dev, const float* mask2_dev, float* y2_dev,
+                                  float* partial_dev, float* y_dev, int N, int H, int W, int Cin, int Cout, int KS, int relu,
+                                  int* launched);
+int dl4ds_op_add_act(const float* a_dev, const float* b_dev, float* out_dev, size_t n, int relu);
+int dl4ds_op_masked_axpy_pair(const float* dy_dev, const float* ya_dev, float* da_dev, const float* yb_dev, float* db_dev,
+                              size_t n, int* launched);
 int dl4ds_op_conv2d_dgrad(const float* dz_dev, const float* w_dev, float* dx_dev, int N, int H, int W,
                           int Cin, int Cout, int KS, int d2s_r, int accumulate);
 int dl4ds_op_conv2d_wgrad(const float* x_dev, const float* dz_dev, float* dw_dev, int N, int H, int W,
```

After: 5268 HR samples/s, median of 6. 1.4% higher.
